# Hongyang-Du/VideoGPA

Hardware: AMD Instinct MI355X
Metric: DPO preference-pair steps/sec, CogVideoX-5B 49f@480x720 (higher is better)
Workload: dtype bf16; 1 GPU; BASELINE configs[1]: CogVideoX-5B T2V full (42 blocks, D=3072, 48x64 heads), 49f x 480x720 -> paired latents [1,2,13,16,60,90], S=17776 tokens, 42 blocks, LoRA r=64 on to_q/to_k/to_v/to_out.0, 1 pair/GPU/step, optimizer step every step; random-init weights; layers=42, pairs_per_gpu=1, parallelism=dp1

## Files before the change

### include/videogpa_hip.h

```cpp
#ifndef VIDEOGPA_HIP_H
#define VIDEOGPA_HIP_H

#include <stddef.h>
#include <stdint.h>

#ifdef __cplusplus
extern "C" {
#endif

typedef struct ihipStream_t* vgpa_stream_t;

#define VGPA_OK 0
#define VGPA_ERR_INVALID (-1)
#define VGPA_ERR_LAUNCH (-2)
#define VGPA_ERR_WORKSPACE (-3)

size_t vgpa_dpo_loss_workspace_bytes(int64_t B);
int32_t vgpa_dpo_loss_fwd(const void* v_win, const void* v_lose, const void* v_win_ref, const void* v_lose_ref,
                          const void* tgt_win, const void* tgt_lose, int64_t B, int64_t N, int64_t stride_pred,
                          int64_t stride_ref, int64_t stride_tgt, int32_t dtype, float beta, float label_smoothing,
                          int32_t loss_type, int32_t flags, float* out5, float* dlogit, float* errs, void* workspace,
                          size_t ws_bytes, vgpa_stream_t stream);
int32_t vgpa_dpo_loss_bwd(const void* v_win, const void* v_lose, const void* tgt_win, const void* tgt_lose, int64_t B,
                          int64_t N, int64_t stride_pred, int64_t stride_tgt, int64_t stride_grad, int32_t dtype, float beta,
                          int32_t flags, const float* dlogit, const float* grad_out, void* grad_win, void* grad_lose,
                          vgpa_stream_t stream);

int32_t vgpa_noise_velocity_paired(const void* x_pair, const void* noise, const int64_t* t, const float* sqrt_abar,
                                   const float* sqrt_1m_abar, int64_t B, int64_t N, int32_t num_train_timesteps,
                                   int32_t dtype, void* x_noisy_pair, void* v_target_pair, vgpa_stream_t stream);

int32_t vgpa_flow_noise_velocity_paired(const void* x_pair, const void* noise, const float* sigma, int64_t B, int64_t N,
                                        int32_t dtype, int32_t xt_f32, void* x_noisy_pair, void* v_target_pair,
                                        vgpa_stream_t stream);

int32_t vgpa_ln_modulate_fwd(const void* x, const float* ln_w, const float* ln_b, const float* shift_v,
                             const float* scale1p_v, const float* shift_t, const float* scale1p_t, int64_t mod_stride,
                             int64_t B, int64_t S, int64_t D, int64_t text_len, float eps, void* out, float* mean,
                             float* rstd, vgpa_stream_t stream);
int32_t vgpa_ln_modulate_bwd(const void* dy, const void* x, const float* mean, const float* rstd, const float* ln_w,
                             const float* scale1p_v, const float* scale1p_t, int64_t mod_stride, int64_t B, int64_t S,
                             int64_t D, int64_t text_len, const void* dres, void* dx, vgpa_stream_t stream);
int32_t vgpa_residual_ln_fwd(const void* x, const void* y, const float* gate_v, const float* gate_t, int64_t gate_stride,
                             const float* ln_w, const float* ln_b, const float* shift_v, const float* scale1p_v,
                             const float* shift_t, const float* scale1p_t, int64_t mod_stride, int64_t B, int64_t S, int64_t D,
                             int64_t text_len, float eps, void* x_new, void* n_out,
                             int64_t n_stride ,
                             float* mean, float* rstd, vgpa_stream_t stream);
int32_t vgpa_residual_ln_bwd(const void* dn, const void* x_new, const float* mean, const float* rstd, const float* ln_w,
                             const float* scale1p_v, const float* scale1p_t, int64_t mod_stride, const float* gate_v,
                             const float* gate_t, int64_t gate_stride, const void* dres, int64_t B, int64_t S, int64_t D,
                             int64_t text_len, void* dx, void* dy, int64_t dy_stride ,
                             vgpa_stream_t stream);
int32_t vgpa_residual_ln_fwd_q8(const void* x, const void* y, const float* gate_v, const float* gate_t, int64_t gate_stride,
                                const float* ln_w, const float* ln_b, const float* shift_v, const float* scale1p_v,
                                const float* shift_t, const float* scale1p_t, int64_t mod_stride, int64_t B, int64_t S, int64_t D,
                                int64_t text_len, float eps, void* x_new, void* q8, float* q8_scale, float* mean, float* rstd,
                                vgpa_stream_t stream);
int32_t vgpa_residual_ln_bwd_q8(const void* dn, const void* x_new, const float* mean, const float* rstd, const float* ln_w,
                                const float* scale1p_v, const float* scale1p_t, int64_t mod_stride, const float* gate_v,
                                const float* gate_t, int64_t gate_stride, const void* dres, int64_t B, int64_t S, int64_t D,
                                int64_t text_len, void* dx, void* dy_q8, float* dy_scale, vgpa_stream_t stream);
int32_t vgpa_gate_residual(const void* x, const void* y, const float* gate_v, const float* gate_t, int64_t mod_stride,
                           int64_t B, int64_t S, int64_t D, int64_t text_len, void* out, vgpa_stream_t stream);
int32_t vgpa_gelu_tanh_fwd(const void* u, int64_t n, void* out, vgpa_stream_t stream);
int32_t vgpa_gelu_tanh_bwd(const void* u, const void* dy, int64_t n, void* du, vgpa_stream_t stream);

int32_t vgpa_qknorm_rope_fwd(const void* q_in, const void* k_in, void* q_out, void* k_out, const int64_t* qin_strides,
                             const int64_t* kin_strides, const int64_t* qout_strides, const int64_t* kout_strides,
                             const float* wq, const float* bq, const float* wk, const float* bk, const float* rope_cos,
                             const float* rope_sin, int64_t text_len, int64_t B, int64_t H, int64_t S, int64_t head_dim,
                             float eps, float q_out_scale, int32_t rope_mode, vgpa_stream_t stream);
int32_t vgpa_qknorm_rope_bwd(const void* dq_out, const void* dk_out, const void* q_in, const void* k_in, void* dq_in,
                             void* dk_in, const int64_t* dqout_strides, const int64_t* dkout_strides,
                             const int64_t* qin_strides, const int64_t* kin_strides, const int64_t* dqin_strides,
                             const int64_t* dkin_strides, const float* wq, const float* wk, const float* rope_cos,
                             const float* rope_sin, int64_t text_len, int64_t B, int64_t H, int64_t S, int64_t head_dim,
                             float eps, int32_t rope_mode, vgpa_stream_t stream);

int32_t vgpa_attn_bwd_delta_res(const void* o, const void* o_res, int32_t res_kind, const void* d_o, const int64_t* o_strides, const int64_t* ores_strides,
                                const int64_t* do_strides, float* delta, int64_t B, int64_t H, int64_t S, int64_t head_dim,
                                vgpa_stream_t stream);
size_t vgpa_attn_bwd_split_workspace_bytes(int64_t B, int64_t H, int64_t S);
int32_t vgpa_attn_bwd_dq_w1(const void* q, const void* k, const void* v, const void* d_o, const float* lse2, const float* delta,
                            void* dq, const int64_t* q_strides, const int64_t* k_strides, const int64_t* v_strides,
                            const int64_t* do_strides, const int64_t* dq_strides, int64_t B, int64_t H, int64_t S, int64_t head_dim,
                            float scale, int32_t split_mode, void* workspace, size_t ws_bytes, vgpa_stream_t stream);
size_t vgpa_attn_fwd_w1_workspace_bytes(int64_t B, int64_t H, int64_t S);
#define VGPA_RES_NONE 0
#define VGPA_RES_BF16 1
#define VGPA_RES_8 2
int32_t vgpa_attn_fwd_w1_res(const void* q, const void* k, const void* v, void* o, void* o_res, int32_t res_kind, float* lse2, const int64_t* q_strides,
                             const int64_t* k_strides, const int64_t* v_strides, const int64_t* o_strides, const int64_t* ores_strides,
                             int64_t B, int64_t H, int64_t S, int64_t head_dim, float scale, int32_t split_mode, void* workspace,
                             size_t ws_bytes, vgpa_stream_t stream);
int32_t vgpa_attn_fwd_online_res(const void* q, const void* k, const void* v, void* o, void* o_res, int32_t res_kind, float* lse2, const int64_t* q_strides,
                                 const int64_t* k_strides, const int64_t* v_strides, const int64_t* o_strides, const int64_t* ores_strides,
                                 int64_t B, int64_t H, int64_t S, int64_t head_dim, float scale, int32_t split_mode, void* workspace,
                                 size_t ws_bytes, vgpa_stream_t stream);
int32_t vgpa_attn_bwd_prep_w1_res(const void* o, const void* o_res, int32_t res_kind, const void* d_o, const float* lse2, const int64_t* o_strides,
                                  const int64_t* ores_strides, const int64_t* do_strides, float* delta, float* stats, int64_t B, int64_t H,
                                  int64_t S, int64_t head_dim, vgpa_stream_t stream);
int32_t vgpa_attn_bwd_dkv_w1(const void* q, const void* k, const void* v, const void* d_o, const float* stats, void* dk, void* dv,
                             const int64_t* q_strides, const int64_t* k_strides, const int64_t* v_strides, const int64_t* do_strides,
                             const int64_t* dk_strides, const int64_t* dv_strides, int64_t B, int64_t H, int64_t S, int64_t head_dim,
                             float scale, int32_t split_mode, void* workspace, size_t ws_bytes, vgpa_stream_t stream);

int32_t vgpa_lora_down(const void* X, int64_t ldx, const void* A, void* T, int64_t ldt, int64_t M, int64_t K, int64_t R,
                       vgpa_stream_t stream);
int32_t vgpa_lora_up_add(void* Y, int64_t ldy, const void* T, int64_t ldt, const void* Bw, int64_t ldb, float s, int64_t M,
                         int64_t N, int64_t rp, int32_t accumulate, vgpa_stream_t stream);
size_t vgpa_lora_grad_workspace_bytes(int64_t M, int64_t P, int64_t Q);
int32_t vgpa_lora_grad_ws(const void* U, int64_t ldu, const void* V, int64_t ldv, float* G, int64_t ldg, float s, int64_t M,
                          int64_t P, int64_t Q, void* workspace, size_t ws_bytes, vgpa_stream_t stream);
int32_t vgpa_lora_ext_refresh(const float* A, const float* B, float s, int64_t r, int64_t K, int64_t Dn, void* a_cat, void* wt_tail, int64_t ld_wt,
                              void* w_tail, int64_t ld_w, void* sbt, vgpa_stream_t stream);

#ifdef VGPA_VARIANTS
int32_t vgpa_gemm_bf16(const void* X, int64_t ldx, const void* W, int64_t ldw, const void* bias, void* C, int64_t ldc, void* aux,
                       int64_t ldaux, int32_t M, int32_t N, int32_t K, int32_t epilogue, vgpa_stream_t stream);
#endif

size_t vgpa_attn128_fwd_workspace_bytes(int64_t B, int64_t H, int64_t Sq);
int32_t vgpa_attn128_fwd(const void* q, const void* k, const void* v, void* o, float* lse2, const int64_t* q_strides, const int64_t* k_strides,
                         const int64_t* v_strides, const int64_t* o_strides, void* o_res8, const int64_t* ores_strides, int64_t B, int64_t H,
                         int64_t Sq, int64_t Skv, float scale, void* workspace, size_t ws_bytes, vgpa_stream_t stream);
size_t vgpa_attn128_fwd_f8_workspace_bytes(int64_t B, int64_t H, int64_t Sq, int64_t Skv);
int32_t vgpa_attn128_fwd_f8(const void* q, const void* k, const void* v, void* o, float* lse2, const int64_t* q_strides, const int64_t* k_strides,
                            const int64_t* v_strides, const int64_t* o_strides, void* o_res8, const int64_t* ores_strides, void* q_deq, void* k_deq,
                            void* v_deq, const int64_t* qd_strides, const int64_t* kd_strides, const int64_t* vd_strides, int64_t B, int64_t H,
                            int64_t Sq, int64_t Skv, float scale, void* workspace, size_t ws_bytes, vgpa_stream_t stream);
size_t vgpa_attn128_bwd_workspace_bytes(int64_t B, int64_t H, int64_t Sq);
int32_t vgpa_attn128_bwd(const void* q, const void* k, const void* v, const void* o, const void* d_o, const float* lse2, void* dq, void* dk,
                         void* dv, const int64_t* q_strides, const int64_t* k_strides, const int64_t* v_strides,
                         const int64_t* o_strides, const int64_t* do_strides, const int64_t* dq_strides, const int64_t* dk_strides,
                         const int64_t* dv_strides, const void* o_res8, const int64_t* ores_strides, int64_t B, int64_t H, int64_t Sq, int64_t Skv,
                         float scale, int32_t dkv_mode, void* workspace, size_t ws_bytes, vgpa_stream_t stream);
int32_t vgpa_attn128_bwd_prescaled(const void* q, const void* k, const void* v, const void* o, const void* d_o, const float* lse2, void* dq, void* dk,
                                   void* dv, const int64_t* q_strides, const int64_t* k_strides, const int64_t* v_strides,
                                   const int64_t* o_strides, const int64_t* do_strides, const int64_t* dq_strides, const int64_t* dk_strides,
                                   const int64_t* dv_strides, const void* o_res8, const int64_t* ores_strides, int64_t B, int64_t H, int64_t Sq, int64_t Skv,
                                   float scale, int32_t dkv_mode, void* workspace, size_t ws_bytes, vgpa_stream_t stream);

int32_t vgpa_wan_ln_mod_fwd(const void* x, int32_t x_dtype, const void* y, const float* gate, float* x_out, const int32_t* gid, const float* ln_w,
                            const float* ln_b, const float* shift, const float* scale, int64_t mod_stride, int64_t rows, int64_t D, float eps,
                            int32_t round_xhat, void* out, int32_t out_dtype, int64_t out_ld, void* q8, float* q8_scale, float* mean, float* rstd,
                            vgpa_stream_t stream);
int32_t vgpa_wan_ln_mod_bwd(const void* dy, int32_t dy_dtype, const void* x, int32_t x_dtype, const float* mean, const float* rstd, const int32_t* gid,
                            const float* ln_w, const float* scale, int64_t mod_stride, int64_t rows, int64_t D, const float* dres, float* dx,
                            const float* gate_prev, void* dy_prev, int64_t ld_dy_prev, vgpa_stream_t stream);
int32_t vgpa_wan_gate_residual(const float* x, const void* y, const int32_t* gid, const float* gate, int64_t mod_stride, int64_t rows, int64_t D, float* out,
                               vgpa_stream_t stream);
int32_t vgpa_wan_gate_bwd(const float* dout, const int32_t* gid, const float* gate, int64_t mod_stride, int64_t rows, int64_t D, void* dy, int64_t ld_dy,
                          vgpa_stream_t stream);
int32_t vgpa_wan_gate_bwd_q8(const float* dout, const int32_t* gid, const float* gate, int64_t mod_stride, int64_t rows, int64_t D, void* q8,
                             float* q8_scale, vgpa_stream_t stream);
int32_t vgpa_wan_rms_rope_fwd(const void* u, int64_t ld_u, const void* w, const float* rope_cos, const float* rope_sin, int64_t L, int64_t head_dim,
                              int64_t rows, int64_t D, float eps, void* out, int64_t ld_out, float* rstd, vgpa_stream_t stream);
int32_t vgpa_wan_rms_rope_bwd(const void* dout, int64_t ld_dout, const void* u, int64_t ld_u, const float* rstd, const void* w, const float* rope_cos,
                              const float* rope_sin, int64_t L, int64_t head_dim, int64_t rows, int64_t D, void* du, int64_t ld_du, vgpa_stream_t stream);

int32_t vgpa_quant_fp8_rows(const void* x, int64_t ldx, void* q, float* scale, int64_t M, int64_t K, vgpa_stream_t stream);
int32_t vgpa_gelu_tanh_fwd_q8(const void* u, int64_t rows, int64_t K, void* q8, float* q8_scale, vgpa_stream_t stream);
int32_t vgpa_gelu_tanh_bwd_q8(const void* u, const void* dy, int64_t rows, int64_t K, void* q8, float* q8_scale, vgpa_stream_t stream);

int32_t vgpa_preprocess_shape(int32_t H, int32_t W, int32_t mode, int32_t* out_h, int32_t* out_w);
size_t vgpa_preprocess_workspace_bytes(int32_t T, int32_t H, int32_t W, int32_t mode);
int32_t vgpa_preprocess_frames(const void* frames, int32_t T, int32_t H, int32_t W, int32_t mode, float* out, void* workspace,
                               size_t ws_bytes, vgpa_stream_t stream);

size_t vgpa_grad_norm_workspace_bytes(void);
int32_t vgpa_grad_norm(const float* grad, int64_t n, float grad_scale, float* norm_out, void* workspace, size_t ws_bytes,
                       vgpa_stream_t stream);
int32_t vgpa_adamw_step(float* param, const float* grad, float* exp_avg, float* exp_avg_sq, int64_t n, float lr, float beta1,
                        float beta2, float eps, float weight_decay, int64_t step, float grad_scale, float max_norm,
                        const float* total_norm, vgpa_stream_t stream);

size_t vgpa_project_points_workspace_bytes(int64_t T, int64_t H, int64_t W);
int32_t vgpa_project_points(const float* pc, const float* colors, const float* conf, float conf_thr,
                            const float* conf_thr_dev , const float* K,
                            const float* E, int32_t e_rows, int64_t N, int64_t T, int64_t H, int64_t W, uint8_t* canvas,
                            float* out_f, void* workspace, size_t ws_bytes, vgpa_stream_t stream);
int32_t vgpa_motion_score(const float* E, int32_t e_rows, int64_t T, float* out, vgpa_stream_t stream);
int32_t vgpa_epipolar_sampson(const float* p1, const float* p2, const int64_t* offsets, int64_t n_pairs, float* err_out,
                              float* F_out, vgpa_stream_t stream);

size_t vgpa_conf_threshold_workspace_bytes(void);
int32_t vgpa_conf_threshold(const float* conf, int64_t N, float conf_thres, float* thr_out, void* workspace, size_t ws_bytes,
                            vgpa_stream_t stream);
size_t vgpa_frame_metric_workspace_bytes(void);
int32_t vgpa_frame_metric(const void* gt, int32_t gt_dtype, int32_t gt_layout, int32_t gt_is_tensor, const void* rep,
                          int32_t rep_dtype, int32_t rep_layout, int32_t rep_is_tensor, int64_t T, int64_t C, int64_t H,
                          int64_t W, int64_t H2, int64_t W2, int32_t psnr, float* out, void* workspace, size_t ws_bytes,
                          vgpa_stream_t stream);
size_t vgpa_frame_ssim_workspace_bytes(int64_t T, int64_t C, int64_t H, int64_t W);
int32_t vgpa_frame_ssim(const void* gt, int32_t gt_dtype, int32_t gt_layout, int32_t gt_is_tensor, const void* rep, int32_t rep_dtype,
                        int32_t rep_layout, int32_t rep_is_tensor, int64_t T, int64_t C, int64_t H, int64_t W, int32_t downsample,
                        float* out_per_frame, float* out_mean, void* workspace, size_t ws_bytes, vgpa_stream_t stream);
int32_t vgpa_frames_to_pm1(const void* src, int32_t dtype, int32_t layout, int32_t is_tensor, int64_t T, int64_t C, int64_t H,
                           int64_t W, int64_t Ho, int64_t Wo, float* out, void* workspace, size_t ws_bytes, vgpa_stream_t stream);
size_t vgpa_mvcs_workspace_bytes(int64_t T);
int32_t vgpa_mvcs(const float* depth, const float* K, int32_t k_dim, const float* E, int32_t e_rows, int64_t T, int64_t H,
                  int64_t W, float* out, void* workspace, size_t ws_bytes, vgpa_stream_t stream);
int32_t vgpa_unproject_depth(const float* depth, const float* K, const float* E, int32_t e_rows, int64_t T, int64_t H,
                             int64_t W, float* world, vgpa_stream_t stream);
int32_t vgpa_pose_decode(const float* pose_enc, int64_t n, float image_h, float image_w, float* ext, float* intr,
                         vgpa_stream_t stream);

int32_t vgpa_conv3x3_f32(const float* x, const float* w_packed, const float* bias, const float* res, const float* res2, float* out,
                         int64_t N, int64_t H, int64_t W, int64_t Cin, int64_t Cout, int64_t stride, int32_t flags,
                         vgpa_stream_t stream);
int32_t vgpa_conv1x1_f32(const float* x, const float* w_packed, const float* bias, float* out, int64_t M, int64_t Cin, int64_t Cout,
                         vgpa_stream_t stream);
int32_t vgpa_dpt_tail_f32(const float* x, const float* xtab, const float* ytab, const float* w1_packed, const float* b1,
                          const float* w2, const float* b2, float* preds, float* conf, int64_t N, int64_t h, int64_t w, int64_t C,
                          int64_t H, int64_t W, int32_t output_dim, int32_t activation, vgpa_stream_t stream);
int32_t vgpa_upsample_bilinear_ac_f32(const float* x, const float* xtab, const float* ytab, float* out, int64_t N, int64_t h,
                                      int64_t w, int64_t C, int64_t H, int64_t W, vgpa_stream_t stream);
int32_t vgpa_attn_small_f32(const float* q, const float* k, const float* v, int64_t stride_b, int64_t stride_h, int64_t stride_s,
                            float* o, int64_t B, int64_t H, int64_t S, int64_t D, float scale, vgpa_stream_t stream);

int32_t vgpa_dino_embed(const void* images, int32_t in_dtype, const float* w_packed, int64_t k_packed, const float* bias,
                        const float* cls_token, const float* register_tokens, const float* pos, void* out, int32_t out_dtype, int64_t N,
                        int64_t H, int64_t W, int64_t patch, int64_t C, int64_t R, vgpa_stream_t stream);
int32_t vgpa_stream_ln_f32(const float* x, const void* y, const float* gamma, const float* ln_w, const float* ln_b, float* x_new, void* n,
                           int32_t n_dtype, int64_t M, int64_t D, float eps, vgpa_stream_t stream);

int32_t vgpa_lpips_input_f32(const float* x, float* out, int64_t N, int64_t H, int64_t W, float shift0, float shift1, float shift2,
                             float scale0, float scale1, float scale2, int32_t flags, vgpa_stream_t stream);
int32_t vgpa_maxpool2x2_f32(const float* x, float* out, int64_t N, int64_t H, int64_t W, int64_t C, int32_t flags, vgpa_stream_t stream);
size_t vgpa_lpips_layer_workspace_bytes(int64_t N, int64_t H, int64_t W, int64_t C);
int32_t vgpa_lpips_layer_f32(const float* f0, const float* f1, const float* w, float* out, double* total, int64_t N, int64_t H, int64_t W,
                             int64_t C, int32_t flags, void* workspace, size_t ws_bytes, vgpa_stream_t stream);

int32_t vgpa_da3_ref_view(const float* x, int64_t B, int64_t S, int64_t N, int64_t C, int32_t strategy, double* metrics, int32_t* ref_idx,
                          vgpa_stream_t stream);
int32_t vgpa_da3_view_gather(const float* a_in, float* a_out, const float* b_in, float* b_out, const int32_t* ref_idx, int32_t inverse, int64_t B,
                             int64_t S, int64_t N, int64_t C, vgpa_stream_t stream);
int32_t vgpa_da3_cam_token(float* x, const float* cam, int32_t per_view, int64_t B, int64_t S, int64_t N, int64_t C, vgpa_stream_t stream);
int32_t vgpa_da3_tap(const float* local_x, const float* x, const float* ln_w, const float* ln_b, float eps, const int32_t* ref_idx, float* feats,
                     float* cam, int64_t B, int64_t S, int64_t N, int64_t C, vgpa_stream_t stream);
int32_t vgpa_da3_pose_decode(const float* pose_enc, int64_t n, float image_h, float image_w, float* ext, float* intr, vgpa_stream_t stream);
int32_t vgpa_dualdpt_aux_tail_f32(const float* x, const float* xtab, const float* ytab, const float* w1_packed, const float* b1,
                                  const float* ln_w, const float* ln_b, float eps, const float* w2, const float* b2, float* preds, float* conf,
                                  int64_t N, int64_t h, int64_t w, int64_t C, int32_t output_dim, vgpa_stream_t stream);

int32_t vgpa_conv3x3_pad_f32(const float* x, const float* w_packed, const float* bias, const float* res, float* out, int64_t N, int64_t H, int64_t W,
                             int64_t Cin, int64_t Cout, int64_t stride, int32_t pad_lo, int32_t pad_hi, vgpa_stream_t stream);
int32_t vgpa_conv3x3x3_causal_f32(const float* x, const float* prev, const float* w_packed, const float* bias, const float* res, float* out, int64_t N,
                                  int64_t T, int64_t H, int64_t W, int64_t Cin, int64_t Cout, vgpa_stream_t stream);
int32_t vgpa_vae_downsample_f32(const float* x, const float* w_packed, const float* bias, float* out, int64_t N, int64_t T, int64_t H, int64_t W,
                                int64_t C, int64_t Cout, int32_t compress_time, vgpa_stream_t stream);
int32_t vgpa_vae_input_f32(const void* x, int32_t in_dtype, float* out, int64_t N, int64_t H, int64_t W, vgpa_stream_t stream);
size_t vgpa_groupnorm_stats_workspace_bytes(int64_t N, int64_t HW, int64_t C, int64_t G);
int32_t vgpa_groupnorm_stats_f32(const float* x, float* stats, int64_t N, int64_t HW, int64_t C, int64_t G, float eps, void* workspace,
                                 size_t ws_bytes, vgpa_stream_t stream);
int32_t vgpa_groupnorm_silu_f32(const float* x, const float* stats, const float* gamma, const float* beta, float* out, int64_t N, int64_t HW,
                                int64_t C, int64_t G, vgpa_stream_t stream);
int32_t vgpa_vae_sample(const float* moments, const void* noise, float scale, void* sample, void* mean, void* logvar, void* std_out,
                        int32_t out_dtype, int64_t N, int64_t hw, int64_t L, vgpa_stream_t stream);

#ifdef __cplusplus
}
#endif
#endif
```

### videogpa_amd/_lib.py

```python
import ctypes
import os

import torch

from ctypes import c_float, c_int32, c_int64, c_size_t, c_void_p

_HERE = os.path.dirname(os.path.abspath(__file__))
LIB_PATH = os.environ.get("VGPA_LIB") or os.path.join(_HERE, "csrc", "libvgpa_hip.so")

P, I64, I32, F32, SZ = c_void_p, c_int64, c_int32, c_float, c_size_t

SIGNATURES = {
    "vgpa_dpo_loss_workspace_bytes": (SZ, [I64]),
    "vgpa_dpo_loss_fwd": (I32, [P, P, P, P, P, P, I64, I64, I64, I64, I64, I32, F32, F32, I32, I32, P, P, P, P, SZ, P]),
    "vgpa_dpo_loss_bwd": (I32, [P, P, P, P, I64, I64, I64, I64, I64, I32, F32, I32, P, P, P, P, P]),
    "vgpa_noise_velocity_paired": (I32, [P, P, P, P, P, I64, I64, I32, I32, P, P, P]),
    "vgpa_flow_noise_velocity_paired": (I32, [P, P, P, I64, I64, I32, I32, P, P, P]),
    "vgpa_ln_modulate_fwd": (I32, [P, P, P, P, P, P, P, I64, I64, I64, I64, I64, F32, P, P, P, P]),
    "vgpa_ln_modulate_bwd": (I32, [P, P, P, P, P, P, P, I64, I64, I64, I64, I64, P, P, P]),
    "vgpa_residual_ln_fwd": (I32, [P, P, P, P, I64, P, P, P, P, P, P, I64, I64, I64, I64, I64, F32, P, P, I64, P, P, P]),
    "vgpa_residual_ln_bwd": (I32, [P, P, P, P, P, P, P, I64, P, P, I64, P, I64, I64, I64, I64, P, P, I64, P]),
    "vgpa_residual_ln_fwd_q8": (I32, [P, P, P, P, I64, P, P, P, P, P, P, I64, I64, I64, I64, I64, F32, P, P, P, P, P, P]),
    "vgpa_residual_ln_bwd_q8": (I32, [P, P, P, P, P, P, P, I64, P, P, I64, P, I64, I64, I64, I64, P, P, P, P]),
    "vgpa_gate_residual": (I32, [P, P, P, P, I64, I64, I64, I64, I64, P, P]),
    "vgpa_gelu_tanh_fwd": (I32, [P, I64, P, P]),
    "vgpa_gelu_tanh_bwd": (I32, [P, P, I64, P, P]),
    "vgpa_qknorm_rope_fwd": (I32, [P, P, P, P, P, P, P, P, P, P, P, P, P, P, I64, I64, I64, I64, I64, F32, F32, I32, P]),
    "vgpa_qknorm_rope_bwd": (I32, [P, P, P, P, P, P, P, P, P, P, P, P, P, P, P, P, I64, I64, I64, I64, I64, F32, I32, P]),
    "vgpa_grad_norm_workspace_bytes": (SZ, []),
    "vgpa_grad_norm": (I32, [P, I64, F32, P, P, SZ, P]),
    "vgpa_adamw_step": (I32, [P, P, P, P, I64, F32, F32, F32, F32, F32, I64, F32, F32, P, P]),
    "vgpa_attn_bwd_delta_res": (I32, [P, P, I32, P, P, P, P, P, I64, I64, I64, I64, P]),
    "vgpa_attn_bwd_dq_w1": (I32, [P, P, P, P, P, P, P, P, P, P, P, P, I64, I64, I64, I64, F32, I32, P, SZ, P]),
    "vgpa_attn_fwd_w1_workspace_bytes": (SZ, [I64, I64, I64]),
    "vgpa_attn_bwd_prep_w1_res": (I32, [P, P, I32, P, P, P, P, P, P, P, I64, I64, I64, I64, P]),
    "vgpa_attn_fwd_w1_res": (I32, [P, P, P, P, P, I32, P, P, P, P, P, P, I64, I64, I64, I64, F32, I32, P, SZ, P]),
    "vgpa_attn_fwd_online_res": (I32, [P, P, P, P, P, I32, P, P, P, P, P, P, I64, I64, I64, I64, F32, I32, P, SZ, P]),
    "vgpa_attn_bwd_dkv_w1": (I32, [P, P, P, P, P, P, P, P, P, P, P, P, P, I64, I64, I64, I64, F32, I32, P, SZ, P]),
    "vgpa_attn_bwd_split_workspace_bytes": (SZ, [I64, I64, I64]),
    "vgpa_lora_down": (I32, [P, I64, P, P, I64, I64, I64, I64, P]),
    "vgpa_lora_up_add": (I32, [P, I64, P, I64, P, I64, F32, I64, I64, I64, I32, P]),
    "vgpa_lora_grad_workspace_bytes": (SZ, [I64, I64, I64]),
    "vgpa_lora_grad_ws": (I32, [P, I64, P, I64, P, I64, F32, I64, I64, I64, P, SZ, P]),
    "vgpa_lora_ext_refresh": (I32, [P, P, F32, I64, I64, I64, P, P, I64, P, I64, P, P]),
    "vgpa_attn128_fwd_workspace_bytes": (SZ, [I64, I64, I64]),
    "vgpa_attn128_fwd": (I32, [P, P, P, P, P, P, P, P, P, P, P, I64, I64, I64, I64, F32, P, SZ, P]),
    "vgpa_attn128_fwd_f8_workspace_bytes": (SZ, [I64, I64, I64, I64]),
    "vgpa_attn128_fwd_f8": (I32, [P] * 17 + [I64, I64, I64, I64, F32, P, SZ, P]),
    "vgpa_attn128_bwd_workspace_bytes": (SZ, [I64, I64, I64]),
    "vgpa_attn128_bwd": (I32, [P] * 19 + [I64, I64, I64, I64, F32, I32, P, SZ, P]),
    "vgpa_attn128_bwd_prescaled": (I32, [P] * 19 + [I64, I64, I64, I64, F32, I32, P, SZ, P]),
    "vgpa_wan_ln_mod_fwd": (I32, [P, I32, P, P, P, P, P, P, P, P, I64, I64, I64, F32, I32, P, I32, I64, P, P, P, P, P]),
    "vgpa_wan_ln_mod_bwd": (I32, [P, I32, P, I32, P, P, P, P, P, I64, I64, I64, P, P, P, P, I64, P]),
    "vgpa_wan_gate_residual": (I32, [P, P, P, P, I64, I64, I64, P, P]),
    "vgpa_wan_gate_bwd": (I32, [P, P, P, I64, I64, I64, P, I64, P]),
    "vgpa_wan_gate_bwd_q8": (I32, [P, P, P, I64, I64, I64, P, P, P]),
    "vgpa_wan_rms_rope_fwd": (I32, [P, I64, P, P, P, I64, I64, I64, I64, F32, P, I64, P, P]),
    "vgpa_wan_rms_rope_bwd": (I32, [P, I64, P, I64, P, P, P, P, I64, I64, I64, I64, P, I64, P]),
    "vgpa_quant_fp8_rows": (I32, [P, I64, P, P, I64, I64, P]),
    "vgpa_gelu_tanh_fwd_q8": (I32, [P, I64, I64, P, P, P]),
    "vgpa_gelu_tanh_bwd_q8": (I32, [P, P, I64, I64, P, P, P]),
    "vgpa_preprocess_shape": (I32, [I32, I32, I32, P, P]),
    "vgpa_preprocess_workspace_bytes": (SZ, [I32, I32, I32, I32]),
    "vgpa_preprocess_frames": (I32, [P, I32, I32, I32, I32, P, P, SZ, P]),
    "vgpa_project_points_workspace_bytes": (SZ, [I64, I64, I64]),
    "vgpa_project_points": (I32, [P, P, P, F32, P, P, P, I32, I64, I64, I64, I64, P, P, P, SZ, P]),
    "vgpa_conf_threshold_workspace_bytes": (SZ, []),
    "vgpa_conf_threshold": (I32, [P, I64, F32, P, P, SZ, P]),
    "vgpa_frame_metric_workspace_bytes": (SZ, []),
    "vgpa_frame_metric": (I32, [P, I32, I32, I32, P, I32, I32, I32, I64, I64, I64, I64, I64, I64, I32, P, P, SZ, P]),
    "vgpa_frame_ssim_workspace_bytes": (SZ, [I64, I64, I64, I64]),
    "vgpa_frame_ssim": (I32, [P, I32, I32, I32, P, I32, I32, I32, I64, I64, I64, I64, I32, P, P, P, SZ, P]),
    "vgpa_frames_to_pm1": (I32, [P, I32, I32, I32, I64, I64, I64, I64, I64, I64, P, P, SZ, P]),
    "vgpa_mvcs_workspace_bytes": (SZ, [I64]),
    "vgpa_mvcs": (I32, [P, P, I32, P, I32, I64, I64, I64, P, P, SZ, P]),
    "vgpa_unproject_depth": (I32, [P, P, P, I32, I64, I64, I64, P, P]),
    "vgpa_pose_decode": (I32, [P, I64, F32, F32, P, P, P]),
    "vgpa_motion_score": (I32, [P, I32, I64, P, P]),
    "vgpa_epipolar_sampson": (I32, [P, P, P, I64, P, P, P]),
    "vgpa_conv3x3_f32": (I32, [P, P, P, P, P, P, I64, I64, I64, I64, I64, I64, I32, P]),
    "vgpa_conv1x1_f32": (I32, [P, P, P, P, I64, I64, I64, P]),
    "vgpa_dpt_tail_f32": (I32, [P, P, P, P, P, P, P, P, P, I64, I64, I64, I64, I64, I64, I32, I32, P]),
    "vgpa_upsample_bilinear_ac_f32": (I32, [P, P, P, P, I64, I64, I64, I64, I64, I64, P]),
    "vgpa_attn_small_f32": (I32, [P, P, P, I64, I64, I64, P, I64, I64, I64, I64, F32, P]),
    "vgpa_dino_embed": (I32, [P, I32, P, I64, P, P, P, P, P, I32, I64, I64, I64, I64, I64, I64, P]),
    "vgpa_stream_ln_f32": (I32, [P, P, P, P, P, P, P, I32, I64, I64, F32, P]),
    "vgpa_lpips_input_f32": (I32, [P, P, I64, I64, I64, F32, F32, F32, F32, F32, F32, I32, P]),
    "vgpa_maxpool2x2_f32": (I32, [P, P, I64, I64, I64, I64, I32, P]),
    "vgpa_lpips_layer_workspace_bytes": (SZ, [I64, I64, I64, I64]),
    "vgpa_lpips_layer_f32": (I32, [P, P, P, P, P, I64, I64, I64, I64, I32, P, SZ, P]),
    "vgpa_da3_ref_view": (I32, [P, I64, I64, I64, I64, I32, P, P, P]),
    "vgpa_da3_view_gather": (I32, [P, P, P, P, P, I32, I64, I64, I64, I64, P]),
    "vgpa_da3_cam_token": (I32, [P, P, I32, I64, I64, I64, I64, P]),
    "vgpa_da3_tap": (I32, [P, P, P, P, F32, P, P, P, I64, I64, I64, I64, P]),
    "vgpa_da3_pose_decode": (I32, [P, I64, F32, F32, P, P, P]),
    "vgpa_dualdpt_aux_tail_f32": (I32, [P, P, P, P, P, P, P, F32, P, P, P, P, I64, I64, I64, I64, I32, P]),
    "vgpa_conv3x3_pad_f32": (I32, [P, P, P, P, P, I64, I64, I64, I64, I64, I64, I32, I32, P]),
    "vgpa_conv3x3x3_causal_f32": (I32, [P, P, P, P, P, P, I64, I64, I64, I64, I64, I64, P]),
    "vgpa_vae_downsample_f32": (I32, [P, P, P, P, I64, I64, I64, I64, I64, I64, I32, P]),
    "vgpa_vae_input_f32": (I32, [P, I32, P, I64, I64, I64, P]),
    "vgpa_groupnorm_stats_workspace_bytes": (SZ, [I64, I64, I64, I64]),
    "vgpa_groupnorm_stats_f32": (I32, [P, P, I64, I64, I64, I64, F32, P, SZ, P]),
    "vgpa_groupnorm_silu_f32": (I32, [P, P, P, P, P, I64, I64, I64, I64, P]),
    "vgpa_vae_sample": (I32, [P, P, F32, P, P, P, P, I32, I64, I64, I64, P]),
}

OPTIONAL_SIGNATURES = {
    "vgpa_gemm_bf16": (I32, [P, I64, P, I64, P, P, I64, P, I64, I32, I32, I32, I32, P]),
}

_ERR = {-1: "invalid argument", -2: "kernel launch failed", -3: "workspace too small"}
_lib = None


def load():
    global _lib
    if _lib is None:
        if not os.path.exists(LIB_PATH):
            raise RuntimeError(
                f"videogpa_amd: HIP library not built ({LIB_PATH} missing). Run `python -m videogpa_amd.build` "
                "(or __graft_entry__.build()). There is no CPU / PyTorch fallback.")
        lib = ctypes.CDLL(LIB_PATH)
        for name, (res, args) in SIGNATURES.items():
            fn = getattr(lib, name)
            fn.restype = res
            fn.argtypes = args
        for name, (res, args) in OPTIONAL_SIGNATURES.items():
            fn = getattr(lib, name, None)
            if fn is not None:
                fn.restype = res
                fn.argtypes = args
        _lib = lib
    return _lib


def _conv(a):
    if a is None:
        return None
    if hasattr(a, "data_ptr"):
        return a.data_ptr()
    return a


def call(name, *args):
    fn = getattr(load(), name)
    rc = fn(*[_conv(a) for a in args])
    if rc != 0:
        raise RuntimeError(f"{name} failed: {_ERR.get(rc, rc)}")


def query(name, *args):
    return getattr(load(), name)(*args)


def has(name):
    return hasattr(load(), name)
```

### videogpa_amd/csrc/attention_w1.hip

```cpp
#include <type_traits>

#include "attn_w1.h"

#define W1_DQ_PART_FLOATS (256 * HD)
#define W1_DKV_PART_FLOATS (2 * 256 * HD)

template <bool SPLIT>
__global__ __launch_bounds__(256, 1) void attn_bwd_dq_w1_kernel(const bf16_t* __restrict__ Q, const bf16_t* __restrict__ K,
                                                                  const bf16_t* __restrict__ V, const bf16_t* __restrict__ dO,
                                                                  const float* __restrict__ LSE2, const float* __restrict__ DELTA,
                                                                  bf16_t* __restrict__ dQ, TStride sq, TStride sk, TStride sv, TStride sdo,
                                                                  TStride sdq, int S, int H, int n_qt, float scale, int task0, int nsplit,
                                                                  float* __restrict__ part) {
    constexpr int QB = 2;
    __shared__ __attribute__((aligned(1024))) uint8_t lds[W1_RING_BYTES];
    int vid, chunk;
    w1_task<SPLIT>(task0, nsplit, vid, chunk);
    const int bh = vid / n_qt, qt = vid % n_qt;
    const int b = bh / H, h = bh % H;
    const int lane = threadIdx.x & 63, hi = lane >> 5;
    const int wave = __builtin_amdgcn_readfirstlane((int)threadIdx.x >> 6);
    const int q0 = (qt * 4 + wave) * (32 * QB);

    bf16x8_t qf[QB][4], dof[QB][4];
    f32x16_t cs[QB], cd[QB];
#pragma unroll
    for (int j = 0; j < QB; ++j) {
        load_row_frags(Q + ((size_t)b * sq.b + (size_t)h * sq.h), sq.s, q0 + 32 * j, S, lane, qf[j]);
        load_row_frags(dO + ((size_t)b * sdo.b + (size_t)h * sdo.h), sdo.s, q0 + 32 * j, S, lane, dof[j]);
        int qc = q0 + 32 * j + (lane & 31);
        qc = qc < S ? qc : S - 1;
        const float nl = -LSE2[(int64_t)bh * S + qc], nd = -DELTA[(int64_t)bh * S + qc];
#pragma unroll
        for (int i = 0; i < 16; ++i) { cs[j][i] = nl; cd[j][i] = nd; }
    }
#pragma unroll
    for (int j = 0; j < QB; ++j) { frags_arrived(qf[j]); frags_arrived(dof[j]); }

    const W1Range tr = w1_split_range(S, chunk, nsplit, SPLIT);
    const int tb = tr.tb, nt = tr.nt;

    w1_zero_slot(lds, 3 * W1_SLOT_BYTES, 2);
    __syncthreads();

    const bf16_t* Kb = K + ((size_t)b * sk.b + (size_t)h * sk.h);
    const bf16_t* Vb = V + ((size_t)b * sv.b + (size_t)h * sv.h);
    const W1Rsrc krs = w1_rsrc(Kb, ((uint32_t)(S - 1) * sk.s + (uint32_t)HD) * 2u);
    const W1Rsrc vrs = w1_rsrc(Vb, ((uint32_t)(S - 1) * sv.s + (uint32_t)HD) * 2u);
    uint32_t kvo[2], vvo[2];
    w1_dma_offsets<HD>(wave, lane, sk.s, kvo);
    w1_dma_offsets<HD>(wave, lane, sv.s, vvo);
    const uint32_t kstep = __builtin_amdgcn_readfirstlane(64u * sk.s * 2u), vstep = __builtin_amdgcn_readfirstlane(64u * sv.s * 2u);
    const uint32_t wbase = __builtin_amdgcn_readfirstlane((uint32_t)(uintptr_t)(__attribute__((address_space(3))) uint8_t*)lds + (uint32_t)wave * 2048u);
    u32x4_t voff = {kvo[0] + (uint32_t)tb * kstep, kvo[1] + (uint32_t)tb * kstep, vvo[0] + (uint32_t)tb * vstep, vvo[1] + (uint32_t)tb * vstep};
    w1_prime<HD>(wbase, krs, vrs, voff, kstep, vstep);

    const u32x8_t la8 = w1_read_offsets<HD>(lane);
    const u32x16_t qf0 = w1_pack4(qf[0][0], qf[0][1], qf[0][2], qf[0][3]), qf1 = w1_pack4(qf[1][0], qf[1][1], qf[1][2], qf[1][3]);
    const u32x16_t do0 = w1_pack4(dof[0][0], dof[0][1], dof[0][2], dof[0][3]), do1 = w1_pack4(dof[1][0], dof[1][1], dof[1][2], dof[1][3]);
    const uint32_t niter = (uint32_t)(nt - tb + 1);
    f32x16_t dq[QB][2];
    uint32_t t0, t1, t2;
    asm volatile(
#include "w1_dq_loop.inc"
        : "=&s"(t0), "=&s"(t1), "=&s"(t2), "={a[0:15]}"(dq[0][0]), "={a[16:31]}"(dq[0][1]), "={a[32:47]}"(dq[1][0]), "={a[48:63]}"(dq[1][1]),
          "+{v[232:235]}"(voff)
        : [rk] "s"(krs.w), [rv] "s"(vrs.w), [kstep] "s"(kstep), [vstep] "s"(vstep), [wbase] "s"(wbase), [niter] "s"(niter), "{a[64:79]}"(qf0),
          "{a[80:95]}"(qf1), "{a[96:111]}"(do0), "{a[112:127]}"(do1), "{v[160:175]}"(cs[0]), "{v[176:191]}"(cs[1]), "{v[192:207]}"(cd[0]), "{v[208:223]}"(cd[1]), "{v[224:231]}"(la8)
        : "memory", "scc",
#include "w1_dq_clobbers.inc"
    );
#pragma unroll
    for (int j = 0; j < QB; ++j) { asm volatile("" : "+v"(dq[j][0])); asm volatile("" : "+v"(dq[j][1])); }

    if (SPLIT) {
        float* pb = part + ((size_t)(vid - task0) * nsplit + chunk) * W1_DQ_PART_FLOATS;
#pragma unroll
        for (int j = 0; j < QB; ++j) {
            const int r = wave * (32 * QB) + 32 * j + (lane & 31);
#pragma unroll
            for (int db = 0; db < 2; ++db)
#pragma unroll
                for (int g = 0; g < 4; ++g) {
                    const f32x4_t w = {dq[j][db][4 * g], dq[j][db][4 * g + 1], dq[j][db][4 * g + 2], dq[j][db][4 * g + 3]};
                    *reinterpret_cast<f32x4_t*>(pb + r * HD + db * 32 + 8 * g + 4 * hi) = w;
                }
        }
        return;
    }
#pragma unroll
    for (int j = 0; j < QB; ++j) {
        const int q = q0 + 32 * j + (lane & 31);
        if (q < S) {
            bf16_t* op = dQ + ((size_t)b * sdq.b + (size_t)h * sdq.h + (size_t)q * sdq.s);
#pragma unroll
            for (int db = 0; db < 2; ++db)
#pragma unroll
                for (int gp = 0; gp < 2; ++gp) {
                    u32x2_t w[2];
#pragma unroll
                    for (int e = 0; e < 2; ++e) {
                        const int g = 2 * gp + e;
                        w[e][0] = pack_bf16x2(dq[j][db][4 * g] * scale, dq[j][db][4 * g + 1] * scale);
                        w[e][1] = pack_bf16x2(dq[j][db][4 * g + 2] * scale, dq[j][db][4 * g + 3] * scale);
                    }
                    *reinterpret_cast<u32x4_t*>(op + db * 32 + 8 * (2 * gp + hi)) = pair_rows8(w[0], w[1]);
                }
        }
    }
}

#include "w1_fwd_knobs.inc"
#define W1_FWD_PART_FLOATS (256 * (HD + 2))
#define W1_FWD_MIN_S 128

__device__ __forceinline__ u32x2_t w1_residual4(const float* x, u32x2_t packed) {
    u32x2_t r;
    r[0] = pack_bf16x2(x[0] - __uint_as_float(packed[0] << 16), x[1] - __uint_as_float(packed[0] & 0xffff0000u));
    r[1] = pack_bf16x2(x[2] - __uint_as_float(packed[1] << 16), x[3] - __uint_as_float(packed[1] & 0xffff0000u));
    return r;
}

template <bool SPLIT>
__global__ __launch_bounds__(256, 1) void attn_fwd_w1_kernel(const bf16_t* __restrict__ Q, const bf16_t* __restrict__ K, const bf16_t* __restrict__ V,
                                                               bf16_t* __restrict__ O, float* __restrict__ LSE2, const unsigned* __restrict__ KMAX2,
                                                               int* __restrict__ flags, TStride sq, TStride sk, TStride sv, TStride so, int S, int H,
                                                               int n_qt, int task0, int nsplit, float* __restrict__ part, void* __restrict__ ORES,
                                                               TStride sor, int res_kind) {
    constexpr int QB = 2;
    __shared__ __attribute__((aligned(1024))) uint8_t lds[W1_RING_BYTES];
    int vid, chunk;
    w1_task<SPLIT>(task0, nsplit, vid, chunk);
    const int bh = vid / n_qt, qt = vid % n_qt;
    const int b = bh / H, h = bh % H;
    const int lane = threadIdx.x & 63, hi = lane >> 5;
    const int wave = __builtin_amdgcn_readfirstlane((int)threadIdx.x >> 6);
    const int q0 = (qt * 4 + wave) * (32 * QB);

    bf16x8_t qf[QB][4];
    float nm[QB];
    const float kmax = sqrtf(__uint_as_float(KMAX2[bh]));
#pragma unroll
    for (int j = 0; j < QB; ++j) load_row_frags(Q + ((size_t)b * sq.b + (size_t)h * sq.h), sq.s, q0 + 32 * j, S, lane, qf[j]);
#pragma unroll
    for (int j = 0; j < QB; ++j) {
        frags_arrived(qf[j]);
        float a = 0.f;
#pragma unroll
        for (int ks = 0; ks < 4; ++ks) {
            float f[8];
            frag_to_f32(qf[j][ks], f);
#pragma unroll
            for (int i = 0; i < 8; ++i) a += f[i] * f[i];
        }
        a += other_half(a);
        nm[j] = sqrtf(a) * kmax * 1.0009765625f;
    }
    {
        const bf16_t* Ks = K + ((size_t)b * sk.b + (size_t)h * sk.h);
        const uint32_t step = (uint32_t)S / W1_SAMPLE_KEYS;
        float ms[QB];
#pragma unroll
        for (int j = 0; j < QB; ++j) ms[j] = -INFINITY;
#pragma unroll
        for (int kb = 0; kb < W1_SAMPLE_KEYS / 32; ++kb) {
            bf16x8_t kf[4];
            load_row_frags(Ks, sk.s * step, 32 * kb, W1_SAMPLE_KEYS, lane, kf);
            frags_arrived(kf);
#pragma unroll
            for (int j = 0; j < QB; ++j) {
                f32x16_t acc = {0.f, 0.f, 0.f, 0.f, 0.f, 0.f, 0.f, 0.f, 0.f, 0.f, 0.f, 0.f, 0.f, 0.f, 0.f, 0.f};
#pragma unroll
                for (int ks = 0; ks < 4; ++ks) acc = mfma32(kf[ks], qf[j][ks], acc);
                float m = acc[0];
#pragma unroll
                for (int i = 1; i < 16; ++i) m = fmaxf(m, acc[i]);
                ms[j] = fmaxf(ms[j], fmaxf(m, other_half(m)));
            }
        }
#pragma unroll
        for (int j = 0; j < QB; ++j) nm[j] = -fminf(nm[j], ms[j] + W1_SAMPLE_UP);
    }

    const W1Range tr = w1_split_range(S, chunk, nsplit, SPLIT);
    const int tb = tr.tb, nt = tr.nt;

    w1_zero_slot(lds, 3 * W1_SLOT_BYTES + W1_TILE_BYTES, 2);
    __syncthreads();

    const bf16_t* Kb = K + ((size_t)b * sk.b + (size_t)h * sk.h);
    const bf16_t* Vb = V + ((size_t)b * sv.b + (size_t)h * sv.h);
    const W1Rsrc krs = w1_rsrc(Kb, ((uint32_t)(S - 1) * sk.s + (uint32_t)HD) * 2u);
    const W1Rsrc vrs = w1_rsrc(Vb, ((uint32_t)(S - 1) * sv.s + (uint32_t)HD) * 2u);
    uint32_t kvo[2], vvo[2];
    w1_dma_offsets<HD>(wave, lane, sk.s, kvo);
    w1_dma_offsets<HD>(wave, lane, sv.s, vvo);
    const uint32_t kstep = __builtin_amdgcn_readfirstlane(64u * sk.s * 2u), vstep = __builtin_amdgcn_readfirstlane(64u * sv.s * 2u);
    const uint32_t wbase = __builtin_amdgcn_readfirstlane((uint32_t)(uintptr_t)(__attribute__((address_space(3))) uint8_t*)lds + (uint32_t)wave * 2048u);
    u32x4_t voff = {kvo[0] + (uint32_t)tb * kstep, kvo[1] + (uint32_t)tb * kstep, vvo[0] + (uint32_t)tb * vstep, vvo[1] + (uint32_t)tb * vstep};
    w1_prime<HD>(wbase, krs, vrs, voff, kstep, vstep);

    const u32x8_t la8 = w1_read_offsets<HD>(lane);
    const u32x16_t qf0 = w1_pack4(qf[0][0], qf[0][1], qf[0][2], qf[0][3]), qf1 = w1_pack4(qf[1][0], qf[1][1], qf[1][2], qf[1][3]);
    const uint32_t niter = (uint32_t)(nt - tb + 1);
    const int kend = nt * TILE < S ? nt * TILE : S;
    const uint32_t krem = (uint32_t)(kend - tb * TILE);
    const uint32_t hi4 = 4u * (uint32_t)hi;
#if W1_FWD_MFSUM
    const uint32_t sel = (lane == 0 || lane == 32 || lane == 17 || lane == 49) ? 0x3f803f80u : 0u;
#define W1_FWD_SEL_IN , "{v158}"(sel)
#else
#define W1_FWD_SEL_IN
#endif
    f32x16_t o[QB][2];
    u32x8_t lv;
    uint32_t t0, t1, t2, t3;
    uint64_t c0, c1;
    asm volatile(
#include "w1_fwd_loop.inc"
        : "=&s"(t0), "=&s"(t1), "=&s"(t2), "=&s"(t3), [c0] "=&s"(c0), [c1] "=&s"(c1), "={a[0:15]}"(o[0][0]), "={a[16:31]}"(o[0][1]), "={a[32:47]}"(o[1][0]), "={a[48:63]}"(o[1][1]),
          "={v[128:135]}"(lv), "+{v[152:155]}"(voff)
        : [rk] "s"(krs.w), [rv] "s"(vrs.w), [kstep] "s"(kstep), [vstep] "s"(vstep), [wbase] "s"(wbase), [niter] "s"(niter), [krem] "s"(krem),
          "{a[64:79]}"(qf0), "{a[80:95]}"(qf1), "{v136}"(nm[0]), "{v137}"(nm[1]), "{v[144:151]}"(la8), "{v156}"(hi4) W1_FWD_SEL_IN
        : "memory", "scc", "vcc",
#include "w1_fwd_clobbers.inc"
    );
#pragma unroll
    for (int j = 0; j < QB; ++j) { asm volatile("" : "+v"(o[j][0])); asm volatile("" : "+v"(o[j][1])); }

    float l[QB];
#pragma unroll
    for (int j = 0; j < QB; ++j) {
#if W1_FWD_MFSUM
        const float s0 = __shfl(__uint_as_float(lv[4 * j]), lane & 15, 64), s1 = __shfl(__uint_as_float(lv[4 * j + 1]), lane & 15, 64);
        l[j] = (lane & 16) ? s1 : s0;
#else
        const float a = (__uint_as_float(lv[4 * j]) + __uint_as_float(lv[4 * j + 1])) + (__uint_as_float(lv[4 * j + 2]) + __uint_as_float(lv[4 * j + 3]));
        l[j] = a + other_half(a);
#endif
    }
    if (SPLIT) {
        float* pb = part + ((size_t)(vid - task0) * nsplit + chunk) * W1_FWD_PART_FLOATS;
#pragma unroll
        for (int j = 0; j < QB; ++j) {
            const int r = wave * (32 * QB) + 32 * j + (lane & 31);
#pragma unroll
            for (int db = 0; db < 2; ++db)
#pragma unroll
                for (int g = 0; g < 4; ++g) {
                    const f32x4_t w = {o[j][db][4 * g], o[j][db][4 * g + 1], o[j][db][4 * g + 2], o[j][db][4 * g + 3]};
                    *reinterpret_cast<f32x4_t*>(pb + r * HD + db * 32 + 8 * g + 4 * hi) = w;
                }
            if (hi == 0) { pb[256 * HD + r] = -nm[j]; pb[256 * HD + 256 + r] = l[j]; }
        }
        return;
    }
    bool bad = false;
#pragma unroll
    for (int j = 0; j < QB; ++j) {
        const int q = q0 + 32 * j + (lane & 31);
        if (q < S) {
            bad = bad || w1_strip_bad(l[j], -nm[j], o[j]);
            const float inv = 1.f / l[j];
            bf16_t* op = O + ((size_t)b * so.b + (size_t)h * so.h + (size_t)q * so.s);
            const size_t ro = (size_t)b * sor.b + (size_t)h * sor.h + (size_t)q * sor.s;
#pragma unroll
            for (int db = 0; db < 2; ++db)
#pragma unroll
                for (int gp = 0; gp < 2; ++gp) {
                    u32x2_t w[2], rw[2];
                    uint32_t rb[2];
#pragma unroll
                    for (int e = 0; e < 2; ++e) {
                        float x[4];
                        w[e] = w1_pack_bf16x4(o[j][db], 2 * gp + e, inv, x);
                        if (res_kind == VGPA_RES_8) rb[e] = res8_pack4(x, w[e]);
                        else if (res_kind == VGPA_RES_BF16) rw[e] = w1_residual4(x, w[e]);
                    }
                    const int d0 = db * 32 + 8 * (2 * gp + hi);
                    *reinterpret_cast<u32x4_t*>(op + d0) = pair_rows8(w[0], w[1]);
                    if (res_kind == VGPA_RES_8) *reinterpret_cast<u32x2_t*>((uint8_t*)ORES + ro + d0) = pair_rows8_dword(rb[0], rb[1]);
                    else if (res_kind == VGPA_RES_BF16) *reinterpret_cast<u32x4_t*>((bf16_t*)ORES + ro + d0) = pair_rows8(rw[0], rw[1]);
                }
            if (hi == 0) LSE2[(int64_t)bh * S + q] = -nm[j] + __builtin_amdgcn_logf(l[j]);
        }
    }
#ifdef W1_CLOCKS
    if (threadIdx.x == 0) flags[vid] = (int)(c1 - c0);
    (void)bad;
#else
    if (__any(bad) && lane == 0) flags[vid] = 1;
#endif
}

__global__ __launch_bounds__(256) void w1_fwd_merge_kernel(const float* __restrict__ part, int nsplit, int task0, int n_qt, bf16_t* __restrict__ O, TStride so,
                                                             float* __restrict__ LSE2, int* __restrict__ flags, int S, int H, void* __restrict__ ORES,
                                                             TStride sor, int res_kind) {
    const int lane = threadIdx.x & 63, r = (blockIdx.x & 63) * 4 + (threadIdx.x >> 6), tl = blockIdx.x >> 6;
    const int vid = task0 + tl, bh = vid / n_qt, qt = vid % n_qt;
    const int q = qt * 256 + r;
    if (q >= S) return;
    const float* pb = part + (size_t)tl * nsplit * W1_FWD_PART_FLOATS;
    float acc = 0.f, L = 0.f;
    for (int c = 0; c < nsplit; ++c) {
        const float* pc = pb + (size_t)c * W1_FWD_PART_FLOATS;
        acc += pc[r * HD + lane];
        L += pc[256 * HD + 256 + r];
    }
    const int b = bh / H, h = bh % H;
    const float x = acc / L;
    const bf16_t xb = f32_to_bf16(x);
    O[(size_t)b * so.b + (size_t)h * so.h + (size_t)q * so.s + lane] = xb;
    const size_t ro = (size_t)b * sor.b + (size_t)h * sor.h + (size_t)q * sor.s + lane;
    if (res_kind == VGPA_RES_8) ((uint8_t*)ORES)[ro] = (uint8_t)res8_byte(x, xb);
    else if (res_kind == VGPA_RES_BF16) ((bf16_t*)ORES)[ro] = f32_to_bf16(x - bf16_to_f32(xb));
    const bool obad = __any(!(fabsf(acc) < INFINITY));
    if (lane == 0) {
        LSE2[(int64_t)bh * S + q] = pb[256 * HD + r] + __builtin_amdgcn_logf(L);
        if (w1_stats_bad(L, pb[256 * HD + r]) || obad) flags[vid] = 1;
    }
}

template <bool SPLIT>
__global__ __launch_bounds__(256, 1) void attn_bwd_dkv_w1_kernel(const bf16_t* __restrict__ Q, const bf16_t* __restrict__ K,
                                                                   const bf16_t* __restrict__ V, const bf16_t* __restrict__ dO,
                                                                   const float* __restrict__ STATS, bf16_t* __restrict__ dK, bf16_t* __restrict__ dV,
                                                                   TStride sq, TStride sk, TStride sv, TStride sdo, TStride sdk, TStride sdv, int S,
                                                                   int H, int n_kt, float kscale, int task0, int nsplit, float* __restrict__ part) {
    constexpr int KB = 2;
    __shared__ __attribute__((aligned(1024))) uint8_t lds[W1_RING_BYTES + W1_SLOTS * W1_STAT_BYTES];
    int vid, chunk;
    w1_task<SPLIT>(task0, nsplit, vid, chunk);
    const int bh = vid / n_kt, kt = vid % n_kt;
    const int b = bh / H, h = bh % H;
    const int lane = threadIdx.x & 63, hi = lane >> 5;
    const int wave = __builtin_amdgcn_readfirstlane((int)threadIdx.x >> 6);
    const int k0 = (kt * 4 + wave) * (32 * KB);

    bf16x8_t kf[KB][4], vf[KB][4];
#pragma unroll
    for (int j = 0; j < KB; ++j) {
        load_row_frags(K + ((size_t)b * sk.b + (size_t)h * sk.h), sk.s, k0 + 32 * j, S, lane, kf[j]);
        load_row_frags(V + ((size_t)b * sv.b + (size_t)h * sv.h), sv.s, k0 + 32 * j, S, lane, vf[j]);
    }
#pragma unroll
    for (int j = 0; j < KB; ++j) { frags_arrived(kf[j]); frags_arrived(vf[j]); }

    const W1Range tr = w1_split_range(S, chunk, nsplit, SPLIT);
    const int tb = tr.tb, nt = tr.nt;

    {
        const u32x4_t z = {0u, 0u, 0u, 0u};
#pragma unroll
        for (int i = 0; i < 4; ++i) *reinterpret_cast<u32x4_t*>(lds + 3 * W1_SLOT_BYTES + i * 4096 + threadIdx.x * 16) = z;
    }
    __syncthreads();

    const bf16_t* Qb = Q + ((size_t)b * sq.b + (size_t)h * sq.h);
    const bf16_t* dOb = dO + ((size_t)b * sdo.b + (size_t)h * sdo.h);
    const W1Rsrc qrs = w1_rsrc(Qb, ((uint32_t)(S - 1) * sq.s + (uint32_t)HD) * 2u);
    const W1Rsrc dors = w1_rsrc(dOb, ((uint32_t)(S - 1) * sdo.s + (uint32_t)HD) * 2u);
    const W1Rsrc strs = w1_rsrc(STATS + (int64_t)bh * 2 * S, (uint32_t)(2 * S) * 4u);
    uint32_t qvo[2], dvo[2];
    w1_dma_offsets<HD>(wave, lane, sq.s, qvo);
    w1_dma_offsets<HD>(wave, lane, sdo.s, dvo);
    const uint32_t qstep = __builtin_amdgcn_readfirstlane(64u * sq.s * 2u), dstep = __builtin_amdgcn_readfirstlane(64u * sdo.s * 2u);
    const uint32_t lds0 = (uint32_t)(uintptr_t)(__attribute__((address_space(3))) uint8_t*)lds;
    const uint32_t wbase = __builtin_amdgcn_readfirstlane(lds0 + (uint32_t)wave * 2048u);
    const uint32_t sbase = __builtin_amdgcn_readfirstlane(lds0 + (uint32_t)W1_RING_BYTES + (uint32_t)wave * 256u);
    const uint32_t srow = (uint32_t)(16 * wave + (lane & 15)), splane = (uint32_t)((lane >> 4) & 1);
    uint32_t svo = (splane * (uint32_t)S + srow + (uint32_t)tb * 64u) * 4u;
    u32x4_t voff = {qvo[0] + (uint32_t)tb * qstep, qvo[1] + (uint32_t)tb * qstep, dvo[0] + (uint32_t)tb * dstep, dvo[1] + (uint32_t)tb * dstep};
#pragma unroll
    for (int i = 0; i < 2; ++i) {
        const uint32_t dst = wbase + (uint32_t)i * W1_SLOT_BYTES;
        w1_dma(dst, qrs, voff[0], 0u);
        w1_dma(dst + 1024u, qrs, voff[1], 0u);
        w1_dma(dst + W1_TILE_BYTES, dors, voff[2], 0u);
        w1_dma(dst + W1_TILE_BYTES + 1024u, dors, voff[3], 0u);
        w1_dma4(sbase + (uint32_t)i * W1_STAT_BYTES, strs, svo, 0u);
        voff[0] += qstep; voff[1] += qstep; voff[2] += dstep; voff[3] += dstep;
        svo += 256u;
    }

    const u32x8_t la8 = w1_read_offsets<HD>(lane);
    const uint32_t sread = lds0 + (uint32_t)W1_RING_BYTES + 16u * (uint32_t)hi;
    const u32x16_t kf0 = w1_pack4(kf[0][0], kf[0][1], kf[0][2], kf[0][3]), kf1 = w1_pack4(kf[1][0], kf[1][1], kf[1][2], kf[1][3]);
    const u32x16_t vf0 = w1_pack4(vf[0][0], vf[0][1], vf[0][2], vf[0][3]), vf1 = w1_pack4(vf[1][0], vf[1][1], vf[1][2], vf[1][3]);
    const uint32_t niter = (uint32_t)(nt - tb + 1);
    f32x16_t dk[KB][2], dv[KB][2];
    uint32_t t0, t1;
    asm volatile(
#include "w1_dkv_loop.inc"
        : "=&s"(t0), "=&s"(t1), "={a[0:15]}"(dk[0][0]), "={a[16:31]}"(dk[0][1]), "={a[32:47]}"(dk[1][0]), "={a[48:63]}"(dk[1][1]),
          "={a[64:79]}"(dv[0][0]), "={a[80:95]}"(dv[0][1]), "={a[96:111]}"(dv[1][0]), "={a[112:127]}"(dv[1][1]), "+{v[232:235]}"(voff), "+{v236}"(svo)
        : [rq] "s"(qrs.w), [rdo] "s"(dors.w), [rst] "s"(strs.w), [qstep] "s"(qstep), [dstep] "s"(dstep), [wbase] "s"(wbase), [sbase] "s"(sbase),
          [niter] "s"(niter), "{a[128:143]}"(kf0), "{a[144:159]}"(kf1), "{a[160:175]}"(vf0), "{a[176:191]}"(vf1), "{v[224:231]}"(la8), "{v237}"(sread)
        : "memory", "scc",
#include "w1_dkv_clobbers.inc"
    );
#pragma unroll
    for (int j = 0; j < KB; ++j)
#pragma unroll
        for (int db = 0; db < 2; ++db) { asm volatile("" : "+v"(dk[j][db])); asm volatile("" : "+v"(dv[j][db])); }

    if (SPLIT) {
        float* pb = part + ((size_t)(vid - task0) * nsplit + chunk) * W1_DKV_PART_FLOATS;
#pragma unroll
        for (int j = 0; j < KB; ++j) {
            const int r = wave * (32 * KB) + 32 * j + (lane & 31);
            w1_store_part_row(pb, r, dk[j], hi);
            w1_store_part_row(pb + 256 * HD, r, dv[j], hi);
        }
        return;
    }
#pragma unroll
    for (int j = 0; j < KB; ++j) {
        const int k = k0 + 32 * j + (lane & 31);
        if (k < S) {
            w1_store_bf16_row(dK + ((size_t)b * sdk.b + (size_t)h * sdk.h + (size_t)k * sdk.s), dk[j], kscale, hi);
            w1_store_bf16_row(dV + ((size_t)b * sdv.b + (size_t)h * sdv.h + (size_t)k * sdv.s), dv[j], 1.f, hi);
        }
    }
}

__global__ __launch_bounds__(256) void w1_dkv_merge_kernel(const float* __restrict__ part, int nsplit, int task0, int n_kt, bf16_t* __restrict__ dK,
                                                             bf16_t* __restrict__ dV, TStride sdk, TStride sdv, int S, int H, float kscale) {
    const int lane = threadIdx.x & 63;
    const int r = ((int)blockIdx.x % 64) * 4 + (threadIdx.x >> 6), tl = (int)blockIdx.x / 64;
    const int vid = task0 + tl, bh = vid / n_kt, kt = vid % n_kt;
    const int key = kt * 256 + r;
    if (key >= S) return;
    const float* pb = part + (size_t)tl * nsplit * W1_DKV_PART_FLOATS + r * HD + lane;
    float ak = 0.f, av = 0.f;
    for (int c = 0; c < nsplit; ++c) {
        ak += pb[(size_t)c * W1_DKV_PART_FLOATS];
        av += pb[(size_t)c * W1_DKV_PART_FLOATS + 256 * HD];
    }
    const int b = bh / H, h = bh % H;
    dK[(size_t)b * sdk.b + (size_t)h * sdk.h + (size_t)key * sdk.s + lane] = f32_to_bf16(ak * kscale);
    dV[(size_t)b * sdv.b + (size_t)h * sdv.h + (size_t)key * sdv.s + lane] = f32_to_bf16(av);
}

__global__ __launch_bounds__(256) void w1_bwd_prep_kernel(const bf16_t* __restrict__ dO, const bf16_t* __restrict__ O, const float* __restrict__ LSE2,
                                                            TStride sdo, TStride so, int S, int H, int64_t total , float* __restrict__ delta,
                                                            float* __restrict__ stats, const void* __restrict__ ORES, TStride sor, int res_kind) {
    const int64_t gid = (int64_t)blockIdx.x * 256 + threadIdx.x;
    const int64_t row = gid >> 3;
    const int c8 = (int)(gid & 7);
    float acc = 0.f;
    int64_t bh = 0;
    int q = 0;
    if (row < total) {
        q = (int)(row % S);
        bh = row / S;
        const int h = (int)(bh % H), b = (int)(bh / H);
        float a[8], o[8];
        unpack8(*reinterpret_cast<const u32x4_t*>(dO + ((size_t)b * sdo.b + (size_t)h * sdo.h + (size_t)q * sdo.s + c8 * 8)), a);
        const u32x4_t ob = *reinterpret_cast<const u32x4_t*>(O + ((size_t)b * so.b + (size_t)h * so.h + (size_t)q * so.s + c8 * 8));
        const size_t ro = (size_t)b * sor.b + (size_t)h * sor.h + (size_t)q * sor.s + c8 * 8;
        if (res_kind == VGPA_RES_8) {
            unpack8_res8(ob, *reinterpret_cast<const u32x2_t*>((const uint8_t*)ORES + ro), o);
        } else {
            unpack8(ob, o);
            if (res_kind == VGPA_RES_BF16) {
                float r[8];
                unpack8(*reinterpret_cast<const u32x4_t*>((const bf16_t*)ORES + ro), r);
#pragma unroll
                for (int j = 0; j < 8; ++j) o[j] += r[j];
            }
        }
#pragma unroll
        for (int j = 0; j < 8; ++j) acc += a[j] * o[j];
    }
    acc += __shfl_xor(acc, 1, 64);
    acc += __shfl_xor(acc, 2, 64);
    acc += __shfl_xor(acc, 4, 64);
    if (row < total && c8 == 0) {
        delta[row] = acc;
        stats[bh * 2 * S + q] = -LSE2[row];
        stats[bh * 2 * S + S + q] = -acc;
    }
}

__global__ __launch_bounds__(256) void w1_dq_merge_kernel(const float* __restrict__ part, int nsplit, int task0, int n_qt, int rows_per_task,
                                                            bf16_t* __restrict__ dQ, TStride sdq, int S, int H, float scale) {
    const int lane = threadIdx.x & 63, rows4 = rows_per_task >> 2;
    const int r = ((int)blockIdx.x % rows4) * 4 + (threadIdx.x >> 6), tl = (int)blockIdx.x / rows4;
    const int vid = task0 + tl, bh = vid / n_qt, qt = vid % n_qt;
    const int q = qt * rows_per_task + r;
    if (q >= S) return;
    const float* pb = part + (size_t)tl * nsplit * rows_per_task * HD + r * HD + lane;
    float acc = 0.f;
    for (int c = 0; c < nsplit; ++c) acc += pb[(size_t)c * rows_per_task * HD];
    const int b = bh / H, h = bh % H;
    dQ[(size_t)b * sdq.b + (size_t)h * sdq.h + (size_t)q * sdq.s + lane] = f32_to_bf16(acc * scale);
}

#define W1_MAX_SPLIT 16
static inline int64_t w1_slots() { return wg_slots() / 2; }

extern "C" {


size_t vgpa_attn_bwd_split_workspace_bytes(int64_t B, int64_t H, int64_t S) {
    if (B <= 0 || H <= 0 || S <= 0) return 0;
    const int64_t tasks = (S + 255) / 256 * B * H;
    const size_t part = W1_DKV_PART_FLOATS > W1_DQ_PART_FLOATS ? W1_DKV_PART_FLOATS : W1_DQ_PART_FLOATS;
    return (size_t)max_split_parts(tasks, W1_MAX_SPLIT, w1_slots()) * part * sizeof(float);
}

int32_t vgpa_attn_bwd_dq_w1(const void* q, const void* k, const void* v, const void* d_o, const float* lse2, const float* delta, void* dq,
                            const int64_t* q_strides, const int64_t* k_strides, const int64_t* v_strides, const int64_t* do_strides,
                            const int64_t* dq_strides, int64_t B, int64_t H, int64_t S, int64_t head_dim, float scale, int32_t split_mode,
                            void* workspace, size_t ws_bytes, hipStream_t stream) {
    if (!q || !k || !v || !d_o || !lse2 || !delta || !dq || head_dim != HD || B <= 0 || H <= 0 || S <= 0 || S > (1 << 24)) return VGPA_ERR_INVALID;
    if (!view_ok(q_strides, B, H, S, HD) || !view_ok(k_strides, B, H, S, HD) || !view_ok(v_strides, B, H, S, HD) || !view_ok(do_strides, B, H, S, HD) ||
        !view_ok(dq_strides, B, H, S, HD) || !al16(q) || !al16(k) || !al16(v) || !al16(d_o) || !al16(dq) || (workspace && !al16(workspace)))
        return VGPA_ERR_INVALID;
    const int rows = 256;
    W1Plan pl;
    const int32_t rc = plan_w1(B, H, S, split_mode, W1_MAX_SPLIT, w1_slots(), W1_DQ_PART_FLOATS * sizeof(float), workspace, ws_bytes, 0, &pl);
    if (rc) return rc;
    const int n_t = pl.n_t;
    const TailSplit& p = pl.p;
    if (p.n_main > 0) {
        VGPA_LAUNCH((attn_bwd_dq_w1_kernel<false>), dim3((unsigned)p.n_main), dim3(256), 0, stream, (const bf16_t*)q, (const bf16_t*)k,
                    (const bf16_t*)v, (const bf16_t*)d_o, lse2, delta, (bf16_t*)dq, mk(q_strides), mk(k_strides), mk(v_strides), mk(do_strides),
                    mk(dq_strides), (int)S, (int)H, n_t, scale, 0, 1, (float*)nullptr);
        VGPA_CHECK_LAUNCH();
    }
    if (p.n_tail > 0) {
        VGPA_LAUNCH((attn_bwd_dq_w1_kernel<true>), dim3((unsigned)(p.n_tail * p.nsplit)), dim3(256), 0, stream, (const bf16_t*)q, (const bf16_t*)k,
                    (const bf16_t*)v, (const bf16_t*)d_o, lse2, delta, (bf16_t*)dq, mk(q_strides), mk(k_strides), mk(v_strides), mk(do_strides),
                    mk(dq_strides), (int)S, (int)H, n_t, scale, (int)p.n_main, p.nsplit, (float*)workspace);
        VGPA_CHECK_LAUNCH();
        VGPA_LAUNCH(w1_dq_merge_kernel, dim3((unsigned)(p.n_tail * (rows / 4))), dim3(256), 0, stream, (const float*)workspace, p.nsplit, (int)p.n_main, n_t,
                    rows, (bf16_t*)dq, mk(dq_strides), (int)S, (int)H, scale);
        VGPA_CHECK_LAUNCH();
    }
    return VGPA_OK;
}


int32_t vgpa_attn_bwd_prep_w1_res(const void* o, const void* o_res, int32_t res_kind, const void* d_o, const float* lse2, const int64_t* o_strides,
                                  const int64_t* ores_strides, const int64_t* do_strides, float* delta, float* stats, int64_t B, int64_t H, int64_t S,
                                  int64_t head_dim, hipStream_t stream) {
    if (!o || !d_o || !lse2 || !delta || !stats || head_dim != HD || B <= 0 || H <= 0 || S <= 0 || S > (1 << 24)) return VGPA_ERR_INVALID;
    if (!view_ok(o_strides, B, H, S, HD) || !view_ok(do_strides, B, H, S, HD) || !al16(o) || !al16(d_o)) return VGPA_ERR_INVALID;
    if (o_res && (!view_ok(ores_strides, B, H, S, HD) || !al16(o_res) || (res_kind != VGPA_RES_BF16 && res_kind != VGPA_RES_8))) return VGPA_ERR_INVALID;
    const int64_t total = B * H * S;
    VGPA_LAUNCH(w1_bwd_prep_kernel, dim3((unsigned)((total * 8 + 255) / 256)), dim3(256), 0, stream, (const bf16_t*)d_o, (const bf16_t*)o, lse2,
                mk(do_strides), mk(o_strides), (int)S, (int)H, total, delta, stats, o_res, o_res ? mk(ores_strides) : mk(o_strides),
                o_res ? (int)res_kind : VGPA_RES_NONE);
    VGPA_CHECK_LAUNCH();
    return VGPA_OK;
}

int32_t vgpa_attn_bwd_dkv_w1(const void* q, const void* k, const void* v, const void* d_o, const float* stats, void* dk, void* dv,
                             const int64_t* q_strides, const int64_t* k_strides, const int64_t* v_strides, const int64_t* do_strides,
                             const int64_t* dk_strides, const int64_t* dv_strides, int64_t B, int64_t H, int64_t S, int64_t head_dim, float scale,
                             int32_t split_mode, void* workspace, size_t ws_bytes, hipStream_t stream) {
    (void)scale;
    if (!q || !k || !v || !d_o || !stats || !dk || !dv || head_dim != HD || B <= 0 || H <= 0 || S <= 0 || S > (1 << 24)) return VGPA_ERR_INVALID;
    if (!view_ok(q_strides, B, H, S, HD) || !view_ok(k_strides, B, H, S, HD) || !view_ok(v_strides, B, H, S, HD) || !view_ok(do_strides, B, H, S, HD) ||
        !view_ok(dk_strides, B, H, S, HD) || !view_ok(dv_strides, B, H, S, HD) || !al16(q) || !al16(k) || !al16(v) || !al16(d_o) || !al16(dk) ||
        !al16(dv) || (workspace && !al16(workspace)))
        return VGPA_ERR_INVALID;
    const float kscale = 0.6931471805599453f;
    W1Plan pl;
    const int32_t rc = plan_w1(B, H, S, split_mode, W1_MAX_SPLIT, w1_slots(), W1_DKV_PART_FLOATS * sizeof(float), workspace, ws_bytes, 0, &pl);
    if (rc) return rc;
    const int n_t = pl.n_t;
    const TailSplit& p = pl.p;
    if (p.n_main > 0) {
        VGPA_LAUNCH((attn_bwd_dkv_w1_kernel<false>), dim3((unsigned)p.n_main), dim3(256), 0, stream, (const bf16_t*)q, (const bf16_t*)k, (const bf16_t*)v,
                    (const bf16_t*)d_o, stats, (bf16_t*)dk, (bf16_t*)dv, mk(q_strides), mk(k_strides), mk(v_strides), mk(do_strides), mk(dk_strides),
                    mk(dv_strides), (int)S, (int)H, n_t, kscale, 0, 1, (float*)nullptr);
        VGPA_CHECK_LAUNCH();
    }
    if (p.n_tail > 0) {
        VGPA_LAUNCH((attn_bwd_dkv_w1_kernel<true>), dim3((unsigned)(p.n_tail * p.nsplit)), dim3(256), 0, stream, (const bf16_t*)q, (const bf16_t*)k,
                    (const bf16_t*)v, (const bf16_t*)d_o, stats, (bf16_t*)dk, (bf16_t*)dv, mk(q_strides), mk(k_strides), mk(v_strides), mk(do_strides),
                    mk(dk_strides), mk(dv_strides), (int)S, (int)H, n_t, kscale, (int)p.n_main, p.nsplit, (float*)workspace);
        VGPA_CHECK_LAUNCH();
        VGPA_LAUNCH(w1_dkv_merge_kernel, dim3((unsigned)(p.n_tail * 64)), dim3(256), 0, stream, (const float*)workspace, p.nsplit, (int)p.n_main, n_t,
                    (bf16_t*)dk, (bf16_t*)dv, mk(dk_strides), mk(dv_strides), (int)S, (int)H, kscale);
        VGPA_CHECK_LAUNCH();
    }
    return VGPA_OK;
}


static inline size_t fwd_w1_ws_head(int64_t B, int64_t H, int64_t tasks) { return (((size_t)(B * H) + (size_t)tasks) * 4 + 255) / 256 * 256; }
size_t vgpa_attn_fwd_w1_workspace_bytes(int64_t B, int64_t H, int64_t S) {
    const int64_t tasks = (S + 255) / 256 * B * H;
    return fwd_w1_ws_head(B, H, tasks) + (size_t)max_split_parts(tasks, W1_MAX_SPLIT, w1_slots()) * W1_FWD_PART_FLOATS * sizeof(float);
}
static int32_t fwd_w1_impl(const void* q, const void* k, const void* v, void* o, void* o_res, int32_t res_kind, float* lse2, const int64_t* q_strides,
                           const int64_t* k_strides, const int64_t* v_strides, const int64_t* o_strides, const int64_t* ores_strides, int64_t B,
                           int64_t H, int64_t S, int64_t head_dim, float scale, int32_t split_mode, void* workspace, size_t ws_bytes,
                           hipStream_t stream, bool force_online) {
    (void)scale;
    if (!q || !k || !v || !o || !lse2 || !workspace || head_dim != HD || B <= 0 || H <= 0 || S <= 0 || S > (1 << 24)) return VGPA_ERR_INVALID;
    if (!view_ok(q_strides, B, H, S, HD) || !view_ok(k_strides, B, H, S, HD) || !view_ok(v_strides, B, H, S, HD) || !view_ok(o_strides, B, H, S, HD) ||
        !al16(q) || !al16(k) || !al16(v) || !al16(o) || !al16(workspace))
        return VGPA_ERR_INVALID;
    if (o_res && (!view_ok(ores_strides, B, H, S, HD) || !al16(o_res) || (res_kind != VGPA_RES_BF16 && res_kind != VGPA_RES_8))) return VGPA_ERR_INVALID;
    void* ores = o_res;
    const int rk = o_res ? (int)res_kind : VGPA_RES_NONE;
    const TStride sor = o_res ? mk(ores_strides) : mk(o_strides);
    if (B * H > 65535) return VGPA_ERR_INVALID;
    const size_t head = fwd_w1_ws_head(B, H, (S + 255) / 256 * B * H);
    W1Plan pl;
    const int32_t rc = plan_w1(B, H, S, force_online ? 0 : split_mode, W1_MAX_SPLIT, w1_slots(), W1_FWD_PART_FLOATS * sizeof(float), workspace, ws_bytes, head, &pl);
    if (rc) return rc;
    if (ws_bytes < head) return VGPA_ERR_WORKSPACE;
    const int n_qt = pl.n_t;
    const int64_t tasks = pl.tasks;
    const TailSplit& p = pl.p;
    unsigned* kmax2 = (unsigned*)workspace;
    int* flags = (int*)workspace + B * H;
    float* part = (float*)((char*)workspace + head);
    if (S < W1_FWD_MIN_S || force_online) {
        if (hipMemsetAsync(workspace, 0xff, head, stream) != hipSuccess) return VGPA_ERR_LAUNCH;
        return vgpa_internal_attn_fwd_redo(q, k, v, o, lse2, mk(q_strides), mk(k_strides), mk(v_strides), mk(o_strides), (int)S, (int)H, n_qt, tasks,
                                           flags, stream, ores, sor, rk);
    }
    if (hipMemsetAsync(workspace, 0, head, stream) != hipSuccess) return VGPA_ERR_LAUNCH;
    VGPA_LAUNCH((w1_kmax_kernel<HD / 8>), dim3(16, (unsigned)(B * H)), dim3(256), 0, stream, (const bf16_t*)k, mk(k_strides), (int)S, (int)H, kmax2);
    VGPA_CHECK_LAUNCH();
    if (p.n_main > 0) {
        VGPA_LAUNCH((attn_fwd_w1_kernel<false>), dim3((unsigned)p.n_main), dim3(256), 0, stream, (const bf16_t*)q, (const bf16_t*)k, (const bf16_t*)v,
                    (bf16_t*)o, lse2, (const unsigned*)kmax2, flags, mk(q_strides), mk(k_strides), mk(v_strides), mk(o_strides), (int)S, (int)H, n_qt, 0, 1,
                    (float*)nullptr, ores, sor, rk);
        VGPA_CHECK_LAUNCH();
    }
    if (p.n_tail > 0) {
        VGPA_LAUNCH((attn_fwd_w1_kernel<true>), dim3((unsigned)(p.n_tail * p.nsplit)), dim3(256), 0, stream, (const bf16_t*)q, (const bf16_t*)k,
                    (const bf16_t*)v, (bf16_t*)o, lse2, (const unsigned*)kmax2, flags, mk(q_strides), mk(k_strides), mk(v_strides), mk(o_strides), (int)S,
                    (int)H, n_qt, (int)p.n_main, p.nsplit, part, ores, sor, rk);
        VGPA_CHECK_LAUNCH();
        VGPA_LAUNCH(w1_fwd_merge_kernel, dim3((unsigned)(p.n_tail * 64)), dim3(256), 0, stream, (const float*)part, p.nsplit, (int)p.n_main, n_qt, (bf16_t*)o,
                    mk(o_strides), lse2, flags, (int)S, (int)H, ores, sor, rk);
        VGPA_CHECK_LAUNCH();
    }
    return vgpa_internal_attn_fwd_redo(q, k, v, o, lse2, mk(q_strides), mk(k_strides), mk(v_strides), mk(o_strides), (int)S, (int)H, n_qt, tasks, flags, stream,
                                       ores, sor, rk);
}
int32_t vgpa_attn_fwd_w1_res(const void* q, const void* k, const void* v, void* o, void* o_res, int32_t res_kind, float* lse2, const int64_t* q_strides,
                             const int64_t* k_strides, const int64_t* v_strides, const int64_t* o_strides, const int64_t* ores_strides, int64_t B,
                             int64_t H, int64_t S, int64_t head_dim, float scale, int32_t split_mode, void* workspace, size_t ws_bytes,
                             hipStream_t stream) {
    return fwd_w1_impl(q, k, v, o, o_res, res_kind, lse2, q_strides, k_strides, v_strides, o_strides, ores_strides, B, H, S, head_dim, scale, split_mode, workspace,
                       ws_bytes, stream, false);
}
int32_t vgpa_attn_fwd_online_res(const void* q, const void* k, const void* v, void* o, void* o_res, int32_t res_kind, float* lse2, const int64_t* q_strides,
                                 const int64_t* k_strides, const int64_t* v_strides, const int64_t* o_strides, const int64_t* ores_strides, int64_t B,
                                 int64_t H, int64_t S, int64_t head_dim, float scale, int32_t split_mode, void* workspace, size_t ws_bytes,
                                 hipStream_t stream) {
    return fwd_w1_impl(q, k, v, o, o_res, res_kind, lse2, q_strides, k_strides, v_strides, o_strides, ores_strides, B, H, S, head_dim, scale, split_mode, workspace,
                       ws_bytes, stream, true);
}

}
```

### videogpa_amd/csrc/qknorm.hip

```cpp
#include "common.h"

struct QStride { int64_t b, h, s; };

__device__ __forceinline__ float group8_sum(float v) {
    v += __shfl_xor(v, 1, 64);
    v += __shfl_xor(v, 2, 64);
    v += __shfl_xor(v, 4, 64);
    return v;
}

__global__ __launch_bounds__(256) void qknorm_rope_fwd_kernel(const bf16_t* __restrict__ q_in, const bf16_t* __restrict__ k_in,
                                                                bf16_t* __restrict__ q_out, bf16_t* __restrict__ k_out, QStride si_q,
                                                                QStride si_k, QStride so_q, QStride so_k, const float* __restrict__ wq,
                                                                const float* __restrict__ bq, const float* __restrict__ wk,
                                                                const float* __restrict__ bk, const float* __restrict__ rope_cos,
                                                                const float* __restrict__ rope_sin, int text_len, int B, int H, int S,
                                                                float eps, float q_out_scale, int rope_mode) {
    const int64_t nvec = (int64_t)B * S * H;
    const int64_t gid = (int64_t)blockIdx.x * 256 + threadIdx.x;
    const int64_t vid = gid >> 3;
    const int c8 = (int)(gid & 7);
    if (vid >= 2 * nvec) return;
    const int which = vid >= nvec;
    uint32_t r = (uint32_t)(which ? vid - nvec : vid);
    const int h = (int)(r % (uint32_t)H); r /= (uint32_t)H;
    const int s = (int)(r % (uint32_t)S);
    const int b = (int)(r / (uint32_t)S);
    const bf16_t* ip = which ? (k_in + b * si_k.b + h * si_k.h + (int64_t)s * si_k.s) : (q_in + b * si_q.b + h * si_q.h + (int64_t)s * si_q.s);
    bf16_t* op = which ? (k_out + b * so_k.b + h * so_k.h + (int64_t)s * so_k.s) : (q_out + b * so_q.b + h * so_q.h + (int64_t)s * so_q.s);
    const float* w = which ? wk : wq;
    const float* bb = which ? bk : bq;
    float x[8];
    unpack8(*reinterpret_cast<const u32x4_t*>(ip + c8 * 8), x);
    float sum = 0.f;
#pragma unroll
    for (int j = 0; j < 8; ++j) sum += x[j];
    const float mean = group8_sum(sum) * (1.f / 64.f);
    float sq = 0.f;
#pragma unroll
    for (int j = 0; j < 8; ++j) { const float d = x[j] - mean; sq += d * d; }
    const float rstd = rsqrtf(group8_sum(sq) * (1.f / 64.f) + eps);
    float y[8];
#pragma unroll
    for (int j = 0; j < 8; ++j) y[j] = (x[j] - mean) * rstd * w[c8 * 8 + j] + bb[c8 * 8 + j];
    if (rope_cos && rope_mode == 1) {
        const bool on = s >= text_len;
        const float* cp = rope_cos + (int64_t)(on ? s - text_len : 0) * 64 + c8 * 8;
        const float* sp = rope_sin + (int64_t)(on ? s - text_len : 0) * 64 + c8 * 8;
        const float sgn = (c8 & 2) ? 1.f : -1.f;
#pragma unroll
        for (int j = 0; j < 8; ++j) {
            const float partner = __shfl_xor(y[j], 2, 64);
            if (on) y[j] = y[j] * cp[j] + sgn * partner * sp[j];
        }
    } else if (rope_cos && s >= text_len) {
        const float* cp = rope_cos + (int64_t)(s - text_len) * 64 + c8 * 8;
        const float* sp = rope_sin + (int64_t)(s - text_len) * 64 + c8 * 8;
#pragma unroll
        for (int j = 0; j < 8; j += 2) {
            const float a = y[j], bq2 = y[j + 1];
            y[j] = a * cp[j] - bq2 * sp[j];
            y[j + 1] = bq2 * cp[j + 1] + a * sp[j + 1];
        }
    }
    if (!which) {
#pragma unroll
        for (int j = 0; j < 8; ++j) y[j] *= q_out_scale;
    }
    *reinterpret_cast<u32x4_t*>(op + c8 * 8) = pack8(y);
}

__global__ __launch_bounds__(256) void qknorm_rope_bwd_kernel(const bf16_t* __restrict__ dq_out, const bf16_t* __restrict__ dk_out,
                                                                const bf16_t* __restrict__ q_in, const bf16_t* __restrict__ k_in,
                                                                bf16_t* __restrict__ dq_in, bf16_t* __restrict__ dk_in, QStride sg_q,
                                                                QStride sg_k, QStride si_q, QStride si_k, QStride sd_q, QStride sd_k,
                                                                const float* __restrict__ wq, const float* __restrict__ wk,
                                                                const float* __restrict__ rope_cos, const float* __restrict__ rope_sin,
                                                                int text_len, int B, int H, int S, float eps, int rope_mode) {
    const int64_t nvec = (int64_t)B * S * H;
    const int64_t gid = (int64_t)blockIdx.x * 256 + threadIdx.x;
    const int64_t vid = gid >> 3;
    const int c8 = (int)(gid & 7);
    if (vid >= 2 * nvec) return;
    const int which = vid >= nvec;
    uint32_t r = (uint32_t)(which ? vid - nvec : vid);
    const int h = (int)(r % (uint32_t)H); r /= (uint32_t)H;
    const int s = (int)(r % (uint32_t)S);
    const int b = (int)(r / (uint32_t)S);
    const QStride sg = which ? sg_k : sg_q, si = which ? si_k : si_q, sd = which ? sd_k : sd_q;
    const bf16_t* gp = (which ? dk_out : dq_out) + b * sg.b + h * sg.h + (int64_t)s * sg.s;
    const bf16_t* ip = (which ? k_in : q_in) + b * si.b + h * si.h + (int64_t)s * si.s;
    bf16_t* op = (which ? dk_in : dq_in) + b * sd.b + h * sd.h + (int64_t)s * sd.s;
    const float* w = which ? wk : wq;
    float g[8], x[8];
    unpack8(*reinterpret_cast<const u32x4_t*>(gp + c8 * 8), g);
    unpack8(*reinterpret_cast<const u32x4_t*>(ip + c8 * 8), x);
    if (rope_cos && rope_mode == 1) {
        const bool on = s >= text_len;
        const int64_t row = (int64_t)(on ? s - text_len : 0) * 64;
        const float* cp = rope_cos + row + c8 * 8;
        const float* spp = rope_sin + row + (c8 ^ 2) * 8;
        const float sgn = (c8 & 2) ? -1.f : 1.f;
#pragma unroll
        for (int j = 0; j < 8; ++j) {
            const float partner = __shfl_xor(g[j], 2, 64);
            if (on) g[j] = g[j] * cp[j] + sgn * partner * spp[j];
        }
    } else if (rope_cos && s >= text_len) {
        const float* cp = rope_cos + (int64_t)(s - text_len) * 64 + c8 * 8;
        const float* sp = rope_sin + (int64_t)(s - text_len) * 64 + c8 * 8;
#pragma unroll
        for (int j = 0; j < 8; j += 2) {
            const float d0 = g[j], d1 = g[j + 1];
            g[j] = d0 * cp[j] + d1 * sp[j + 1];
            g[j + 1] = d1 * cp[j + 1] - d0 * sp[j];
        }
    }
    float sum = 0.f;
#pragma unroll
    for (int j = 0; j < 8; ++j) sum += x[j];
    const float mean = group8_sum(sum) * (1.f / 64.f);
    float sq = 0.f;
#pragma unroll
    for (int j = 0; j < 8; ++j) { x[j] -= mean; sq += x[j] * x[j]; }
    const float rstd = rsqrtf(group8_sum(sq) * (1.f / 64.f) + eps);
    float s1 = 0.f, s2 = 0.f;
#pragma unroll
    for (int j = 0; j < 8; ++j) {
        x[j] *= rstd;
        g[j] *= w[c8 * 8 + j];
        s1 += g[j];
        s2 += g[j] * x[j];
    }
    const float c1 = group8_sum(s1) * (1.f / 64.f), c2 = group8_sum(s2) * (1.f / 64.f);
#pragma unroll
    for (int j = 0; j < 8; ++j) g[j] = rstd * (g[j] - c1 - x[j] * c2);
    *reinterpret_cast<u32x4_t*>(op + c8 * 8) = pack8(g);
}

static inline bool qs_ok(const int64_t* st) { return st && (st[0] % 8 == 0) && (st[1] % 8 == 0) && (st[2] % 8 == 0); }
static inline QStride qmk(const int64_t* st) { QStride t; t.b = st[0]; t.h = st[1]; t.s = st[2]; return t; }

extern "C" {

int32_t vgpa_qknorm_rope_fwd(const void* q_in, const void* k_in, void* q_out, void* k_out, const int64_t* qin_strides,
                             const int64_t* kin_strides, const int64_t* qout_strides, const int64_t* kout_strides, const float* wq,
                             const float* bq, const float* wk, const float* bk, const float* rope_cos, const float* rope_sin,
                             int64_t text_len, int64_t B, int64_t H, int64_t S, int64_t head_dim, float eps, float q_out_scale,
                             int32_t rope_mode, hipStream_t stream) {
    if (!q_in || !k_in || !q_out || !k_out || !wq || !bq || !wk || !bk || head_dim != 64 || B <= 0 || H <= 0 || S <= 0) return VGPA_ERR_INVALID;
    if (!qs_ok(qin_strides) || !qs_ok(kin_strides) || !qs_ok(qout_strides) || !qs_ok(kout_strides)) return VGPA_ERR_INVALID;
    if ((rope_cos == nullptr) != (rope_sin == nullptr) || text_len < 0 || text_len > S || (rope_mode != 0 && rope_mode != 1)) return VGPA_ERR_INVALID;
    const int64_t threads = 2 * B * S * H * 8;
    if (2 * B * S * H >= ((int64_t)1 << 31) || threads / 256 >= ((int64_t)1 << 31)) return VGPA_ERR_INVALID;
    VGPA_LAUNCH(qknorm_rope_fwd_kernel, dim3((unsigned)((threads + 255) / 256)), dim3(256), 0, stream, (const bf16_t*)q_in,
                       (const bf16_t*)k_in, (bf16_t*)q_out, (bf16_t*)k_out, qmk(qin_strides), qmk(kin_strides), qmk(qout_strides),
                       qmk(kout_strides), wq, bq, wk, bk, rope_cos, rope_sin, (int)text_len, (int)B, (int)H, (int)S, eps, q_out_scale, (int)rope_mode);
    VGPA_CHECK_LAUNCH();
    return VGPA_OK;
}

int32_t vgpa_qknorm_rope_bwd(const void* dq_out, const void* dk_out, const void* q_in, const void* k_in, void* dq_in, void* dk_in,
                             const int64_t* dqout_strides, const int64_t* dkout_strides, const int64_t* qin_strides,
                             const int64_t* kin_strides, const int64_t* dqin_strides, const int64_t* dkin_strides, const float* wq,
                             const float* wk, const float* rope_cos, const float* rope_sin, int64_t text_len, int64_t B, int64_t H,
                             int64_t S, int64_t head_dim, float eps, int32_t rope_mode, hipStream_t stream) {
    if (!dq_out || !dk_out || !q_in || !k_in || !dq_in || !dk_in || !wq || !wk || head_dim != 64 || B <= 0 || H <= 0 || S <= 0) return VGPA_ERR_INVALID;
    if (!qs_ok(dqout_strides) || !qs_ok(dkout_strides) || !qs_ok(qin_strides) || !qs_ok(kin_strides) || !qs_ok(dqin_strides) || !qs_ok(dkin_strides))
        return VGPA_ERR_INVALID;
    if ((rope_cos == nullptr) != (rope_sin == nullptr) || text_len < 0 || text_len > S || (rope_mode != 0 && rope_mode != 1)) return VGPA_ERR_INVALID;
    const int64_t threads = 2 * B * S * H * 8;
    if (2 * B * S * H >= ((int64_t)1 << 31) || threads / 256 >= ((int64_t)1 << 31)) return VGPA_ERR_INVALID;
    VGPA_LAUNCH(qknorm_rope_bwd_kernel, dim3((unsigned)((threads + 255) / 256)), dim3(256), 0, stream, (const bf16_t*)dq_out,
                       (const bf16_t*)dk_out, (const bf16_t*)q_in, (const bf16_t*)k_in, (bf16_t*)dq_in, (bf16_t*)dk_in, qmk(dqout_strides),
                       qmk(dkout_strides), qmk(qin_strides), qmk(kin_strides), qmk(dqin_strides), qmk(dkin_strides), wq, wk, rope_cos,
                       rope_sin, (int)text_len, (int)B, (int)H, (int)S, eps, (int)rope_mode);
    VGPA_CHECK_LAUNCH();
    return VGPA_OK;
}

}
```

### videogpa_amd/ops.py

```python
import contextlib as _contextlib
import contextvars as _contextvars
import ctypes
import os as _os

import torch

from . import _lib

_DT = {torch.float32: 0, torch.bfloat16: 1}


def _stream():
    return torch.cuda.current_stream().cuda_stream


def _req(t, dtype=None, contiguous=True):
    if not t.is_cuda:
        raise RuntimeError("videogpa_amd ops need GPU tensors (no CPU fallback)")
    if dtype is not None and t.dtype != dtype:
        raise RuntimeError(f"expected {dtype}, got {t.dtype}")
    if contiguous and not t.is_contiguous():
        raise RuntimeError("expected a contiguous tensor")
    return t

# ... 613 lines not shown
    M, K = x2.shape
    q = torch.empty(M, K, dtype=torch.float8_e4m3fn, device=x2.device)
    sc = torch.empty(M, 1, dtype=torch.float32, device=x2.device)
    _timed("quant_fp8_rows", 3.0 * M * K, lambda: _lib.call("vgpa_quant_fp8_rows", x2, x2.stride(0), q, sc, M, K, _stream()), "byte")
    return q, sc


def gelu_tanh_fwd_q8(u2):
    M, K = u2.shape
    q = torch.empty(M, K, dtype=torch.float8_e4m3fn, device=u2.device)
    sc = torch.empty(M, 1, dtype=torch.float32, device=u2.device)
    _timed("gelu_tanh_fwd_q8", 3.0 * M * K, lambda: _lib.call("vgpa_gelu_tanh_fwd_q8", u2, M, K, q, sc, _stream()), "byte")
    return q, sc


def gelu_tanh_bwd_q8(u2, dy2):
    M, K = u2.shape
    q = torch.empty(M, K, dtype=torch.float8_e4m3fn, device=u2.device)
    sc = torch.empty(M, 1, dtype=torch.float32, device=u2.device)
    _timed("gelu_tanh_bwd_q8", 5.0 * M * K, lambda: _lib.call("vgpa_gelu_tanh_bwd_q8", u2, dy2, M, K, q, sc, _stream()), "byte")
    return q, sc


class Fp8Weight:

    def __init__(self, W):
        self.version = W._version
        self.q, self.s = self._rows(W.detach())
        self.qt, self.st = self._rows(W.detach().t().contiguous())

    @staticmethod
    def _rows(w):
        fmax = torch.finfo(torch.float8_e4m3fn).max
        amax = w.float().abs().amax(dim=1, keepdim=True)
        sc = torch.where(amax > 0, amax / fmax, torch.ones_like(amax))
        return (w.float() / sc).clamp(-fmax, fmax).to(torch.float8_e4m3fn), sc.t().contiguous()

    @staticmethod
    def of(W):
        c = getattr(W, "_vgpa_fp8", None)
        if c is None or c.version != W._version or c.q.device != W.device:
            c = Fp8Weight(W)
            W._vgpa_fp8 = c
        return c


def _fp8_gemm(xq, sx, wq, sw, bias=None):
    M, N, K = xq.shape[0], wq.shape[0], xq.shape[1]
    out = []

    _timed("hipblaslt_gemm_fp8 (vendor)", 2.0 * M * N * K,
           lambda: out.append(torch._scaled_mm(xq, wq.t(), scale_a=sx, scale_b=sw, bias=bias, out_dtype=torch.bfloat16)))
    return out[0]


class _Fp8FrozenLinearFn(torch.autograd.Function):
    @staticmethod
    def forward(ctx, x, W, bias):
        w8 = Fp8Weight.of(W)
        x2 = x.reshape(-1, x.shape[-1])
        if x2.stride(1) != 1:
            x2 = x2.contiguous()
        xq, sx = quant_fp8_rows(x2)
        ctx.w8 = w8
        return _fp8_gemm(xq, sx, w8.q, w8.s, bias).view(*x.shape[:-1], W.shape[0])

    @staticmethod
    def backward(ctx, dy):
        w8 = ctx.w8
        dy2 = dy.reshape(-1, dy.shape[-1])
        if dy2.stride(1) != 1:
            dy2 = dy2.contiguous()
        dq, sd = quant_fp8_rows(dy2)
        return _fp8_gemm(dq, sd, w8.qt, w8.st).view(*dy.shape[:-1], w8.qt.shape[0]), None, None


def frozen_linear_fp8(x, W, bias):
    if W.requires_grad or (bias is not None and bias.requires_grad):
        raise RuntimeError("videogpa_amd: the fp8 path is for frozen projections only")
    if x.dtype != torch.bfloat16:
        raise TypeError("frozen_linear_fp8: bf16 activations")
    return _Fp8FrozenLinearFn.apply(x, W, bias)


class _FfnTailFp8Fn(torch.autograd.Function):

    @staticmethod
    def forward(ctx, x, a, gates1, ln_w, ln_b, mod2, W1, b1, W2, b2, gates2, nxt_w, nxt_b, nxt_mod, nxt_eps, text_len, eps, n_pad, dy_pad):
        _req(x, torch.bfloat16), _req(a, torch.bfloat16), _req(gates1, torch.float32), _req(gates2, torch.float32)
        _req(ln_w, torch.float32), _req(ln_b, torch.float32), _req(nxt_w, torch.float32), _req(nxt_b, torch.float32)
        B, S, D = x.shape
        rows, dev = B * S, x.device
        keep = any(ctx.needs_input_grad)
        w1, w2 = Fp8Weight.of(W1), Fp8Weight.of(W2)
        x1 = torch.empty_like(x)
        hq = torch.empty(rows, D, dtype=torch.float8_e4m3fn, device=dev)
        hs = torch.empty(rows, 1, dtype=torch.float32, device=dev)
        mean1 = torch.empty(B, S, dtype=torch.float32, device=dev) if keep else None
        rstd1 = torch.empty_like(mean1) if keep else None
        sv, s1v, st, s1t, mstride = _mod_ptrs(mod2)
        _timed("residual_ln_fwd_fp8", 7.0 * rows * D,
               lambda: _lib.call("vgpa_residual_ln_fwd_q8", x, a, gates1[:, 0], gates1[:, 1], gates1.stride(0), ln_w, ln_b, sv, s1v, st, s1t, mstride,
                                 B, S, D, text_len, float(eps), x1, hq, hs, mean1, rstd1, _stream()), "byte")
        u = _fp8_gemm(hq, hs, w1.q, w1.s, b1)
        del hq, hs
        gq, gs = gelu_tanh_fwd_q8(u)
        f = _fp8_gemm(gq, gs, w2.q, w2.s, b2)
        del gq, gs
        x2 = torch.empty_like(x)
        n = _padded_empty((B, S), D, n_pad, x.dtype, dev) if n_pad else _empty_rows(x.shape, x.dtype, dev)
        mean2 = torch.empty(B, S, dtype=torch.float32, device=dev) if keep else None
        rstd2 = torch.empty_like(mean2) if keep else None
        nv, n1v, nt, n1t, nstride = _mod_ptrs(nxt_mod)
        _timed("residual_ln_fwd", 8.0 * rows * D,
               lambda: _lib.call("vgpa_residual_ln_fwd", x1, f, gates2[:, 0], gates2[:, 1], gates2.stride(0), nxt_w, nxt_b, nv, n1v, nt, n1t, nstride,
                                 B, S, D, text_len, float(nxt_eps), x2, n, D + n_pad, mean2, rstd2, _stream()), "byte")
        if keep:
            ctx.save_for_backward(x1, mean1, rstd1, u, x2, mean2, rstd2, ln_w, mod2, gates1, nxt_w, nxt_mod, gates2)
            ctx.w, ctx.text_len, ctx.dy_pad = (w1, w2), text_len, dy_pad
        return x2, n

    @staticmethod
    def backward(ctx, dx2, dn):
        x1, mean1, rstd1, u, x2, mean2, rstd2, ln_w, mod2, gates1, nxt_w, nxt_mod, gates2 = ctx.saved_tensors
        w1, w2 = ctx.w
        B, S, D = x1.shape
        rows, dev = B * S, x1.device
        dn = torch.zeros_like(x2) if dn is None else dn.contiguous()
        dres = None if dx2 is None else dx2.contiguous()
        dx1 = torch.empty_like(x1)
        dfq = torch.empty(rows, D, dtype=torch.float8_e4m3fn, device=dev)
        dfs = torch.empty(rows, 1, dtype=torch.float32, device=dev)
        _, n1v, _, n1t, nstride = _mod_ptrs(nxt_mod)
        _timed("residual_ln_bwd_fp8", (7.0 + (2.0 if dres is not None else 0.0)) * rows * D,
               lambda: _lib.call("vgpa_residual_ln_bwd_q8", dn, x2, mean2, rstd2, nxt_w, n1v, n1t, nstride, gates2[:, 0], gates2[:, 1], gates2.stride(0),
                                 dres, B, S, D, ctx.text_len, dx1, dfq, dfs, _stream()), "byte")
        dg = _fp8_gemm(dfq, dfs, w2.qt, w2.st)
        del dfq, dfs
        duq, dus = gelu_tanh_bwd_q8(u, dg)
        del dg
        dh = _fp8_gemm(duq, dus, w1.qt, w1.st)
        del duq, dus
        dx = torch.empty_like(x1)
        dyp = ctx.dy_pad
        da = _padded_empty((B, S), D, dyp, x1.dtype, dev) if dyp else _empty_rows(x1.shape, x1.dtype, dev)
        _, s1v, _, s1t, mstride = _mod_ptrs(mod2)
        _timed("residual_ln_bwd", 10.0 * rows * D,
               lambda: _lib.call("vgpa_residual_ln_bwd", dh, x1, mean1, rstd1, ln_w, s1v, s1t, mstride, gates1[:, 0], gates1[:, 1], gates1.stride(0),
                                 dx1, B, S, D, ctx.text_len, dx, da, D + dyp, _stream()), "byte")
        return (dx, da) + (None,) * 17


def ffn_tail_fp8(x, a, gates1, ln_w, ln_b, mod2, W1, b1, W2, b2, gates2, nxt_w, nxt_b, nxt_mod=None, nxt_eps=1e-5, text_len=0, eps=1e-5, n_pad=0, dy_pad=0):
    if W1.requires_grad or W2.requires_grad or (b1 is not None and b1.requires_grad) or (b2 is not None and b2.requires_grad):
        raise RuntimeError("videogpa_amd: the fp8 path is for frozen projections only")
    if W1.shape[0] > 16384:
        raise RuntimeError(f"ffn_tail_fp8: the GELU -> e4m3 kernels hold one feed-forward row per workgroup, inner <= 16384; got {W1.shape[0]}")
    return _FfnTailFp8Fn.apply(x, a, gates1, ln_w, ln_b, mod2, W1, b1, W2, b2, gates2, nxt_w, nxt_b, nxt_mod, nxt_eps, int(text_len), eps, int(n_pad),
                               int(dy_pad))


class _LinearLoraExtFn(torch.autograd.Function):

    @staticmethod
    def forward(ctx, x, bias, ext, enabled, scalings, x_recompute, *AB):
        K, R, N = ext.K, ext.R, ext.N
        x2 = x.reshape(-1, K)
        M = x2.shape[0]
        x_ext = _padded_base(x2, K + R)
        if x_ext is None:
            x_ext = torch.zeros(M, K + R, dtype=x.dtype, device=x.device) if not enabled else torch.empty(M, K + R, dtype=x.dtype, device=x.device)
            x_ext[:, :K].copy_(x2)
        xv, tv = x_ext[:, :K], x_ext[:, K:]
        if enabled:
            lora_down(xv, ext.A_cat, out=tv)
        ctx.rows_per_call = current_gemm_rows()
        y = _gemm(x_ext, ext.W_ext, bias, ext=True, split=ctx.rows_per_call)
        if x_recompute is not None and enabled:
            fn, srcs = x_recompute
            ctx.save_for_backward(tv.contiguous(), *srcs)
            ctx.x_fn = fn
        else:
            ctx.save_for_backward(x_ext)
            ctx.x_fn = None
        ctx.ext, ctx.enabled, ctx.xshape, ctx.scalings = ext, enabled, x.shape, scalings
        return y.view(*x.shape[:-1], N)

    @staticmethod
    def backward(ctx, dy):
        ext, enabled = ctx.ext, ctx.enabled
        saved, *srcs = ctx.saved_tensors
        K, R, N, Dn, rp, r, act = ext.K, ext.R, ext.N, ext.Dn, ext.rp, ext.r, ext.act
        dy2 = dy.reshape(-1, N)
        M = dy2.shape[0]
        dy_ext = _padded_base(dy2, N + R) if dy2.stride(1) == 1 else None
        if dy_ext is None:
            dy_ext = torch.zeros(M, N + R, dtype=dy.dtype, device=dy.device) if not enabled else torch.empty(M, N + R, dtype=dy.dtype, device=dy.device)
            dy_ext[:, :N].copy_(dy2)
        if enabled:
            for j, i in enumerate(act):
                lora_down(dy_ext[:, i * Dn:(i + 1) * Dn], ext.sBt[j], out=dy_ext[:, N + j * rp:N + (j + 1) * rp])
        dx = _gemm(dy_ext, ext.Wt_ext, ext=True, split=ctx.rows_per_call)
        out_grads = [None] * len(ctx.needs_input_grad[6:])
        if enabled:
            if ctx.x_fn is not None:
                t_all, xh = saved, ctx.x_fn(*srcs).reshape(M, K)
            else:
                t_all, xh = saved[:, K:], saved[:, :K]
            for j, i in enumerate(act):
                out_grads[2 * i + 1] = lora_grad(dy_ext[:, i * Dn:(i + 1) * Dn], t_all[:, j * rp:(j + 1) * rp], ctx.scalings[j])[:, :r]
            dA = lora_grad(dy_ext[:, N:], xh)
            for j, i in enumerate(act):
                out_grads[2 * i] = dA[j * rp:j * rp + r]
        return (dx.view(ctx.xshape), None, None, None, None, None, *out_grads)


def linear_lora_ext(x, W, bias, ext, loras, enabled=True, x_recompute=None):
    if W.requires_grad or (bias is not None and bias.requires_grad):
        raise RuntimeError("videogpa_amd: base weights are frozen on this path (LoRA-only training, as in the reference)")
    ext.refresh(W, len(loras), loras)
    flat = []
    for l in loras:
        flat += [None, None] if l is None else [l[0], l[1]]
    return _LinearLoraExtFn.apply(x, bias, ext, bool(enabled), tuple(float(loras[i][2]) for i in ext.act), x_recompute, *flat)


def linear_lora(x, W, bias, loras, ext=None):
    if all(l is None for l in loras):
        return frozen_linear(x, W, bias)
    if ext is None:
        ext = getattr(W, "_vgpa_lora_ext", None)
        if ext is None:
            ext = LoraExt()
            W._vgpa_lora_ext = ext
    return linear_lora_ext(x, W, bias, ext, loras, True)


def _bhs_strides(t):
    assert t.stride(3) == 1
    return _i64x3(t.stride(0), t.stride(1), t.stride(2))


LOG2E = 1.4426950408889634
ATTN_SPLIT_MODE = -1
def precise_delta_default():
    v = _os.environ.get("VGPA_PRECISE_DELTA", "int8").lower()
    if v in ("0", "off", "none", "false"):
        return None
    if v in ("1", "int8", "res8", "true"):
        return "int8"
    if v == "bf16":
        return "bf16"
    raise ValueError(f"VGPA_PRECISE_DELTA={v!r}: expected 0 | off | int8 | bf16")


def _res_kind(o_res):
    if o_res is None:
        return 0
    if o_res.dtype == torch.bfloat16:
        return 1
    if o_res.dtype == torch.uint8:
        return 2
    raise TypeError(f"o_res: bf16 (rounding residual) or uint8 (eight further mantissa bits), got {o_res.dtype}")


def res8_decode(o, o_res8):
    E = (o.contiguous().view(torch.int16).to(torch.int32) >> 7) & 0xFF
    sc = torch.where(E > 15, torch.ldexp(torch.ones((), device=o.device), E - 142), torch.zeros((), device=o.device))
    return o.float() + (o_res8.float() - 128.0) * sc


def prescale_q(q, scale=None):
    scale = q.shape[-1] ** -0.5 if scale is None else scale
    return (q.float() * (scale * LOG2E)).to(q.dtype)


class AttnFwdPolicy:
    SWITCH, CHECKS, RECHECK = 0.5, 2, 1024

    def __init__(self, mode="bound", fixed=False):
        self.mode, self.fixed = mode, fixed
        self.calls = 0
        self.redo_fraction = None
        self.switched_at = None

    def wants_flags(self):
        return self.mode == "bound" and not self.fixed and (self.calls < self.CHECKS or self.calls % self.RECHECK == 0)

    def observe(self, fraction):
        self.redo_fraction = fraction
        if not self.fixed and fraction > self.SWITCH:
            self.mode, self.switched_at = "online", self.calls


def _strip_flags(ws, head_words, B, H, Sq):
    strips = (Sq + 255) // 256
    return ws[:4 * (head_words + B * H * strips)].view(torch.int32)[head_words:].view(B, H, strips)


def attention_redo_fraction(ws, B, H, S):
    return float((_strip_flags(ws, B * H, B, H, S) != 0).float().mean())


def attention_fwd_raw(q, k, v, scale=None, q_prescaled=False, split_mode=None, o_pad=0, o_res=None, policy=None):
    B, H, S, Dh = q.shape
    scale = Dh ** -0.5 if scale is None else scale
    if not q_prescaled:
        q = prescale_q(q, scale)
    o = _padded_empty((B, S), H * Dh, o_pad, torch.bfloat16, q.device) if o_pad else torch.empty(B, S, H * Dh, dtype=torch.bfloat16, device=q.device)
    lse = torch.empty(B, H, S, dtype=torch.float32, device=q.device)
    ov = o.unflatten(-1, (H, Dh)).permute(0, 2, 1, 3)
    split_mode = ATTN_SPLIT_MODE if split_mode is None else split_mode
    ws_bytes = _lib.query("vgpa_attn_fwd_w1_workspace_bytes", B, H, S)
    ws = torch.empty(ws_bytes, dtype=torch.uint8, device=q.device)
    rv = None if o_res is None else o_res.unflatten(-1, (H, Dh)).permute(0, 2, 1, 3)
    entry = "vgpa_attn_fwd_online_res" if (policy is not None and policy.mode == "online") else "vgpa_attn_fwd_w1_res"
    _timed("attn_fwd_kernel", 4.0 * S * S * Dh * B * H, lambda: _lib.call(
        entry, q, k, v, o, o_res, _res_kind(o_res), lse, _bhs_strides(q), _bhs_strides(k), _bhs_strides(v), _bhs_strides(ov), None if rv is None else _bhs_strides(rv),
        B, H, S, Dh, float(scale), int(split_mode), ws, ws_bytes, _stream()))
    if policy is not None:
        if policy.wants_flags() and not torch.cuda.is_current_stream_capturing():
            policy.observe(attention_redo_fraction(ws, B, H, S))
        policy.calls += 1
    return o, lse


def attention_bwd_raw(q, k, v, o, do, lse, dq, dk, dv, scale=None, q_prescaled=False, split_mode=None, o_res=None):
    B, H, S, Dh = q.shape
    scale = Dh ** -0.5 if scale is None else scale
    if not q_prescaled:
        q = prescale_q(q, scale)
    delta = torch.empty(B, H, S, dtype=torch.float32, device=q.device)
    st = _stream()
    stats = torch.empty(B, H, 2, S, dtype=torch.float32, device=q.device)
    _timed("attn_delta_kernel", (4.0 + (0 if o_res is None else o_res.element_size())) * B * H * S * Dh, lambda: _lib.call(
        "vgpa_attn_bwd_prep_w1_res", o, o_res, _res_kind(o_res), do, lse, _bhs_strides(o), None if o_res is None else _bhs_strides(o_res), _bhs_strides(do),
        delta, stats, B, H, S, Dh, st), "byte")
    split_mode = ATTN_SPLIT_MODE if split_mode is None else split_mode
    ws_bytes = _lib.query("vgpa_attn_bwd_split_workspace_bytes", B, H, S) if split_mode != 0 else 0
    ws = torch.empty(max(ws_bytes, 16), dtype=torch.uint8, device=q.device)
    wsp = ws if ws_bytes else None
    _timed("attn_bwd_dkv_kernel", 6.0 * S * S * Dh * B * H, lambda: _lib.call(
        "vgpa_attn_bwd_dkv_w1", q, k, v, do, stats, dk, dv, _bhs_strides(q), _bhs_strides(k), _bhs_strides(v), _bhs_strides(do),
        _bhs_strides(dk), _bhs_strides(dv), B, H, S, Dh, float(scale), int(split_mode), wsp, ws_bytes, st))
    _timed("attn_bwd_dq_kernel", 2.0 * S * S * Dh * B * H, lambda: _lib.call(
        "vgpa_attn_bwd_dq_w1", q, k, v, do, lse, delta, dq, _bhs_strides(q), _bhs_strides(k), _bhs_strides(v), _bhs_strides(do),
        _bhs_strides(dq), B, H, S, Dh, float(scale), int(split_mode), wsp, ws_bytes, st))


ATTN128_W1 = True


ATTN128_F8_MIN_KEYS = 1024


def attention128_uses_f8(f8, Skv):
    return bool(f8) and Skv >= ATTN128_F8_MIN_KEYS


class F8AttnPolicy:
    ERR_PER_BOUND = 0.004

    def __init__(self, mode="f8", fixed=False, threshold=0.5):
        self.mode, self.fixed, self.threshold = mode, fixed, float(threshold)
        self.decided = False
        self.estimated_score_error = None

    def reset(self):
        self.decided = False

    @staticmethod
    def score_error_estimate(q, k, H, scale):
        B, Lq, D = q.shape
        d = D // H
        qn = q.view(B, Lq, H, d).float().pow(2).sum(-1).amax(dim=1).sqrt()
        kn = k.view(B, k.shape[1], H, d).float().pow(2).sum(-1).amax(dim=1).sqrt()
        return float((qn * kn).amax()) * float(scale) * LOG2E * F8AttnPolicy.ERR_PER_BOUND

    def use_f8(self, q, k, H, scale):
        if not self.fixed and not self.decided and self.mode == "f8":
            self.estimated_score_error = self.score_error_estimate(q, k, H, scale)
            if self.estimated_score_error > self.threshold:
                self.mode = "bf16"
        self.decided = True
        return self.mode == "f8"


def attention128_f8_redo_fraction(ws, B, H, Sq):
    return float((_strip_flags(ws, 5 * B * H, B, H, Sq) != 0).float().mean())


def attention128_fwd_raw(q, k, v, scale, o_pad=0, f8=False, o_res8=None, deq=None, report=None):
    B, H, Sq, D = q.shape
    Skv = k.shape[2]
    assert D == 128 and k.shape == (B, H, Skv, 128) and v.shape == k.shape and q.dtype == k.dtype == v.dtype == torch.bfloat16
    o2 = _padded_empty((B, Sq), H * D, o_pad, torch.bfloat16, q.device) if o_pad else torch.empty(B, Sq, H * D, dtype=torch.bfloat16, device=q.device)
    o = o2.unflatten(-1, (H, D)).permute(0, 2, 1, 3)
    lse = torch.empty(B, H, Sq, dtype=torch.float32, device=q.device)
    rv = rs = None
    if o_res8 is not None:
        if o_res8.dtype != torch.uint8 or o_res8.shape != (B, Sq, H * D) or not o_res8.is_contiguous():
            raise TypeError("attention128_fwd_raw: o_res8 is a contiguous uint8 [B, Sq, H*128] buffer")
        rv = o_res8.unflatten(-1, (H, D)).permute(0, 2, 1, 3)
        rs = _bhs_strides(rv)
    if attention128_uses_f8(f8, Skv):
        ws_bytes = _lib.query("vgpa_attn128_fwd_f8_workspace_bytes", B, H, Sq, Skv)
        ws = torch.empty(ws_bytes, dtype=torch.uint8, device=q.device)
        dv_ = [None] * 3
        if deq is not None:
            for t, S_ in zip(deq, (Sq, Skv, Skv)):
                if t.dtype != torch.bfloat16 or t.shape != (B, S_, H * D) or not t.is_contiguous():
                    raise TypeError("attention128_fwd_raw: deq = three contiguous bf16 [B, S, H*128] buffers (q, k, v)")
            dv_ = [t.unflatten(-1, (H, D)).permute(0, 2, 1, 3) for t in deq]
        ds_ = [None if t is None else _bhs_strides(t) for t in dv_]
        _timed("attn128_fwd_f8", 4.0 * B * H * Sq * Skv * D, lambda: _lib.call(
            "vgpa_attn128_fwd_f8", q, k, v, o, lse, _bhs_strides(q), _bhs_strides(k), _bhs_strides(v), _bhs_strides(o), rv, rs, dv_[0], dv_[1], dv_[2],
            ds_[0], ds_[1], ds_[2], B, H, Sq, Skv, float(scale), ws, ws_bytes, _stream()))
        if report is not None:
            report["redo_fraction"] = attention128_f8_redo_fraction(ws, B, H, Sq)
            report["strip_flags"] = _strip_flags(ws, 5 * B * H, B, H, Sq) != 0
        return o, lse
    if deq is not None:
        raise ValueError("attention128_fwd_raw: deq buffers are written by the e4m3 forward only (f8=True and at least ATTN128_F8_MIN_KEYS keys)")
    ws_bytes = _lib.query("vgpa_attn128_fwd_workspace_bytes", B, H, Sq) if ATTN128_W1 else 0
    ws = torch.empty(ws_bytes, dtype=torch.uint8, device=q.device) if ws_bytes else None
    _timed("attn128_fwd" if Skv >= 1024 else "attn128_fwd (short keys)", 4.0 * B * H * Sq * Skv * D, lambda: _lib.call(
        "vgpa_attn128_fwd", q, k, v, o, lse, _bhs_strides(q), _bhs_strides(k), _bhs_strides(v), _bhs_strides(o), rv, rs, B, H, Sq, Skv, float(scale),
        ws, ws_bytes, _stream()))
    return o, lse


def attention128_bwd_raw(q, k, v, o, do, lse, dq, dk, dv, scale, o_res8=None, q_prescaled=False):
    B, H, Sq, D = q.shape
    Skv = k.shape[2]
    rv = None if o_res8 is None else o_res8.unflatten(-1, (H, D)).permute(0, 2, 1, 3)
    ws_bytes = _lib.query("vgpa_attn128_bwd_workspace_bytes", B, H, Sq)
    ws = torch.empty(ws_bytes, dtype=torch.uint8, device=q.device)
    _timed("attn128_bwd" if Skv >= 1024 else "attn128_bwd (short keys)", 8.0 * B * H * Sq * Skv * D, lambda: _lib.call(
        "vgpa_attn128_bwd_prescaled" if q_prescaled else "vgpa_attn128_bwd", q, k, v, o, do, lse, dq, dk, dv, _bhs_strides(q), _bhs_strides(k), _bhs_strides(v), _bhs_strides(o), _bhs_strides(do),
        _bhs_strides(dq), _bhs_strides(dk), _bhs_strides(dv), rv, None if rv is None else _bhs_strides(rv), B, H, Sq, Skv, float(scale),
        -1 if ATTN128_W1 else 0, ws, ws_bytes, _stream()))


class _Attention128Fn(torch.autograd.Function):

    @staticmethod
    def forward(ctx, q, k, v, scale, o_pad, precise_delta):
        q, k, v = (t if t.stride(3) == 1 else t.contiguous() for t in (q, k, v))
        o_res8 = None
        if precise_delta and any(ctx.needs_input_grad[:3]):
            o_res8 = torch.empty(q.shape[0], q.shape[2], q.shape[1] * q.shape[3], dtype=torch.uint8, device=q.device)
        o, lse = attention128_fwd_raw(q, k, v, scale, o_pad, o_res8=o_res8)
        ctx.save_for_backward(q, k, v, o, lse, o_res8)
        ctx.scale = float(scale)
        return o

    @staticmethod
    def backward(ctx, do):
        q, k, v, o, lse, o_res8 = ctx.saved_tensors
        B, H, Sq, D = q.shape
        Skv = k.shape[2]
        do = do if do.stride(3) == 1 else do.contiguous()
        dq = torch.empty(B, Sq, H, D, dtype=torch.bfloat16, device=q.device).permute(0, 2, 1, 3)
        dk = torch.empty(B, Skv, H, D, dtype=torch.bfloat16, device=q.device).permute(0, 2, 1, 3)
        dv = torch.empty(B, Skv, H, D, dtype=torch.bfloat16, device=q.device).permute(0, 2, 1, 3)
        attention128_bwd_raw(q, k, v, o, do, lse, dq, dk, dv, ctx.scale, o_res8=o_res8)
        return dq, dk, dv, None, None, None


def attention128(q, k, v, scale=None, o_pad=0, precise_delta="int8"):
    if precise_delta not in (None, "int8"):
        raise ValueError('attention128: precise_delta is "int8" or None (the bf16 residual form exists at head_dim 64 only)')
    return _Attention128Fn.apply(q, k, v, q.shape[-1] ** -0.5 if scale is None else scale, int(o_pad), precise_delta)


class _QKNormAttentionFn(torch.autograd.Function):

    @staticmethod
    def forward(ctx, qkv, wq, bq, wk, bk, rope_cos, rope_sin, text_len, H, eps, o_pad, grad_pad, rope_mode=0, recompute_qk=False, precise_delta=None, fwd_policy=None):
        _req(qkv, torch.bfloat16)
        B, S, W = qkv.shape
        Dh = W // (3 * H)
        qkv5 = qkv.view(B, S, 3, H, Dh)
        q_in, k_in, v = (qkv5[:, :, i].permute(0, 2, 1, 3) for i in range(3))
        qn = torch.empty(B, H, S, Dh, dtype=torch.bfloat16, device=qkv.device)
        kn = torch.empty_like(qn)
        _timed("qknorm_rope_fwd", 8.0 * B * H * S * Dh, lambda: _lib.call(
            "vgpa_qknorm_rope_fwd", q_in, k_in, qn, kn, _bhs_strides(q_in), _bhs_strides(k_in), _bhs_strides(qn), _bhs_strides(kn),
            wq, bq, wk, bk, rope_cos, rope_sin, text_len, B, H, S, Dh, float(eps), float(Dh ** -0.5 * LOG2E), int(rope_mode), _stream()), "byte")
        o_res = None
        if precise_delta and ctx.needs_input_grad[0]:
            o_res = torch.empty(B, S, H * Dh, dtype=torch.uint8 if precise_delta == "int8" else torch.bfloat16, device=qkv.device)
        o, lse = attention_fwd_raw(qn, kn, v, q_prescaled=True, o_pad=o_pad, o_res=o_res, policy=fwd_policy)
        if recompute_qk:
            ctx.save_for_backward(qkv, o, lse, wq, wk, rope_cos, rope_sin, bq, bk, o_res)
        else:
            ctx.save_for_backward(qkv, qn, kn, o, lse, wq, wk, rope_cos, rope_sin, o_res)
        ctx.meta = (text_len, H, eps, grad_pad, int(rope_mode), bool(recompute_qk))
        return o

    @staticmethod
    def backward(ctx, do):
        text_len, H, eps, grad_pad, rope_mode, recompute_qk = ctx.meta
        if recompute_qk:
            qkv, o, lse, wq, wk, rope_cos, rope_sin, bq, bk, o_res = ctx.saved_tensors
        else:
            qkv, qn, kn, o, lse, wq, wk, rope_cos, rope_sin, o_res = ctx.saved_tensors
        B, S, W = qkv.shape
        Dh = W // (3 * H)
        do = do.contiguous()
        qkv5 = qkv.view(B, S, 3, H, Dh)
        q_in, k_in, v = (qkv5[:, :, i].permute(0, 2, 1, 3) for i in range(3))
        if recompute_qk:
            qn = torch.empty(B, H, S, Dh, dtype=torch.bfloat16, device=qkv.device)
            kn = torch.empty_like(qn)
            _timed("qknorm_rope_fwd", 8.0 * B * H * S * Dh, lambda: _lib.call(
                "vgpa_qknorm_rope_fwd", q_in, k_in, qn, kn, _bhs_strides(q_in), _bhs_strides(k_in), _bhs_strides(qn), _bhs_strides(kn),
                wq, bq, wk, bk, rope_cos, rope_sin, text_len, B, H, S, Dh, float(eps), float(Dh ** -0.5 * LOG2E), int(rope_mode), _stream()), "byte")
        dqkv = _padded_empty((B, S), W, grad_pad, qkv.dtype, qkv.device) if grad_pad else torch.empty_like(qkv)
        d5 = dqkv.unflatten(-1, (3, H, Dh))
        dq_in, dk_in, dv = (d5[:, :, i].permute(0, 2, 1, 3) for i in range(3))
        dqn = torch.empty_like(qn)
        dkn = torch.empty_like(kn)
        ov = o.unflatten(-1, (H, Dh)).permute(0, 2, 1, 3)
        dov = do.view(B, S, H, Dh).permute(0, 2, 1, 3)
        attention_bwd_raw(qn, kn, v, ov, dov, lse, dqn, dkn, dv, q_prescaled=True,
                          o_res=None if o_res is None else o_res.unflatten(-1, (H, Dh)).permute(0, 2, 1, 3))
        _timed("qknorm_rope_bwd", 12.0 * B * H * S * Dh, lambda: _lib.call(
            "vgpa_qknorm_rope_bwd", dqn, dkn, q_in, k_in, dq_in, dk_in, _bhs_strides(dqn), _bhs_strides(dkn), _bhs_strides(q_in),
            _bhs_strides(k_in), _bhs_strides(dq_in), _bhs_strides(dk_in), wq, wk, rope_cos, rope_sin, text_len, B, H, S, Dh,
            float(eps), rope_mode, _stream()), "byte")
        return dqkv, None, None, None, None, None, None, None, None, None, None, None, None, None, None, None


def qknorm_attention(qkv, wq, bq, wk, bk, H, text_len=0, rope=None, eps=1e-6, o_pad=0, grad_pad=0, rope_mode=0, recompute_qk=False, precise_delta="int8", fwd_policy=None):
    cos, sin = (None, None) if rope is None else rope
    if precise_delta not in (None, "int8", "bf16"):
        raise ValueError(f'precise_delta: "int8", "bf16" or None, got {precise_delta!r}')
    return _QKNormAttentionFn.apply(qkv, wq, bq, wk, bk, cos, sin, text_len, H, eps, o_pad, grad_pad, rope_mode, bool(recompute_qk), precise_delta, fwd_policy)


def rope2d_tables(pos, head_dim=64, frequency=100.0):
    half = head_dim // 2
    inv = 1.0 / (frequency ** (torch.arange(0, half, 2, device=pos.device).float() / half))
    ang = pos.float()[:, :, None] * inv[None, None, :]
    ang = torch.cat([ang, ang], dim=-1).reshape(pos.shape[0], head_dim)
    return ang.cos().contiguous(), ang.sin().contiguous()


def _heads_in(*ts):
    for t in ts:
        if t is None:
            continue
        _req(t, torch.float32)
        if torch.is_grad_enabled() and t.requires_grad:
            raise RuntimeError("the fp32 head kernels are forward only: call them under torch.no_grad()")


def pack_conv_weight(w):
    return w.detach().float().permute(2, 3, 1, 0).contiguous()


def conv3x3_f32(x, w_packed, bias=None, res=None, res2=None, relu_in=False, relu_res=False, stride=1):
    _heads_in(x, w_packed, bias, res, res2)
    N, H, W, Cin = x.shape
    Cout = w_packed.shape[-1]
    if tuple(w_packed.shape) != (3, 3, Cin, Cout) or Cin % 16 or Cout % 16:
        raise RuntimeError(f"conv3x3_f32: weight {tuple(w_packed.shape)} does not fit input channels {Cin} (multiples of 16)")
    Ho, Wo = (H - 1) // stride + 1, (W - 1) // stride + 1
    out = torch.empty(N, Ho, Wo, Cout, device=x.device, dtype=torch.float32)
    for r in (res, res2):
        if r is not None and r.shape != out.shape:
            raise RuntimeError("conv3x3_f32: residual shape differs from the output's")
    _timed("conv3x3_f32", 2.0 * out.numel() * 9 * Cin,
           lambda: _lib.call("vgpa_conv3x3_f32", x, w_packed, bias, res, res2, out, N, H, W, Cin, Cout, stride,
                             (1 if relu_in else 0) | (2 if relu_res else 0), _stream()))
    return out


def conv1x1_f32(x, w_packed, bias=None):
    _heads_in(x, w_packed, bias)
    Cin, Cout = w_packed.shape
    if x.shape[-1] != Cin or Cin % 16 or Cout % 16:
        raise RuntimeError(f"conv1x1_f32: weight {tuple(w_packed.shape)} does not fit input {tuple(x.shape)} (channels in multiples of 16)")
    out = torch.empty(*x.shape[:-1], Cout, device=x.device, dtype=torch.float32)
    M = out.numel() // Cout
    _timed("conv1x1_f32", 2.0 * M * Cin * Cout, lambda: _lib.call("vgpa_conv1x1_f32", x, w_packed, bias, out, M, Cin, Cout, _stream()))
    return out


def uv_embed_tables(width, height, channels, aspect_ratio, device, ratio=0.1, f32_angles=False):
    if channels % 8:
        raise RuntimeError("uv_embed_tables: channels must be a multiple of 8")
    diag = (aspect_ratio ** 2 + 1.0) ** 0.5
    span_x, span_y = aspect_ratio / diag, 1.0 / diag
    xs = torch.linspace(-span_x * (width - 1) / width, span_x * (width - 1) / width, steps=width, dtype=torch.float32)
    ys = torch.linspace(-span_y * (height - 1) / height, span_y * (height - 1) / height, steps=height, dtype=torch.float32)
    half = channels // 2
    adt = torch.float32 if f32_angles else torch.float64
    omega = torch.arange(half // 2, dtype=adt)
    omega /= half / 2.0
    omega = 1.0 / 100 ** omega

    def table(pos):
        ang = torch.einsum("m,d->md", pos.to(adt), omega)
        return (torch.cat([ang.sin(), ang.cos()], dim=1).float() * ratio).contiguous().to(device)
    return table(xs), table(ys)


def upsample_bilinear_ac_f32(x, H, W, tabs=None):
    xt, yt = tabs if tabs is not None else (None, None)
    _heads_in(x, xt, yt)
    N, h, w, C = x.shape
    if xt is not None and (tuple(xt.shape) != (W, C // 2) or tuple(yt.shape) != (H, C // 2)):
        raise RuntimeError("upsample_bilinear_ac_f32: embedding tables do not fit the output")
    out = torch.empty(N, H, W, C, device=x.device, dtype=torch.float32)
    _timed("upsample_bilinear_ac_f32", 4.0 * out.numel(), lambda: _lib.call("vgpa_upsample_bilinear_ac_f32", x, xt, yt, out, N, h, w, C, H, W, _stream()),
           unit="byte")
    return out


_DPT_ACT = {"exp": 0, "inv_log": 1}


def _tail_fits(name, x, H, W, w1_packed, w2, xt, yt, grid):
    C, od = x.shape[3], w2.shape[0]
    if tuple(w1_packed.shape) != (3, 3, C, 32) or tuple(w2.shape) != (od, 32) or C % 16:
        raise RuntimeError(f"{name}: weights do not fit the input")
    if xt is not None and (tuple(xt.shape) != (W, C // 2) or tuple(yt.shape) != (H, C // 2)):
        raise RuntimeError(f"{name}: embedding tables do not fit the {grid}")


def dpt_tail_f32(x, H, W, w1_packed, b1, w2, b2, activation="exp", tabs=None):
    xt, yt = tabs if tabs is not None else (None, None)
    _heads_in(x, xt, yt, w1_packed, b1, w2, b2)
    if activation not in _DPT_ACT:
        raise NotImplementedError(f"dpt_tail_f32: activation {activation!r} (exp and inv_log are built)")
    N, h, w, C = x.shape
    od = w2.shape[0]
    _tail_fits("dpt_tail_f32", x, H, W, w1_packed, w2, xt, yt, "output")
    preds = torch.empty(N, H, W, od - 1, device=x.device, dtype=torch.float32)
    conf = torch.empty(N, H, W, device=x.device, dtype=torch.float32)
    _timed("dpt_tail_f32", 2.0 * N * H * W * (9 * C * 32 + 32 * od),
           lambda: _lib.call("vgpa_dpt_tail_f32", x, xt, yt, w1_packed, b1, w2, b2, preds, conf, N, h, w, C, H, W, od, _DPT_ACT[activation], _stream()))
    return preds, conf


def dualdpt_aux_tail_f32(x, w1_packed, b1, ln_w, ln_b, eps, w2, b2, tabs=None):
    xt, yt = tabs if tabs is not None else (None, None)
    _heads_in(x, xt, yt, w1_packed, b1, ln_w, ln_b, w2, b2)
    N, h, w, C = x.shape
    od = w2.shape[0]
    if not 2 <= od <= 8:
        raise RuntimeError("dualdpt_aux_tail_f32: weights do not fit the input")
    _tail_fits("dualdpt_aux_tail_f32", x, h, w, w1_packed, w2, xt, yt, "map")
    if b1.numel() != 32 or ln_w.numel() != 32 or ln_b.numel() != 32 or b2.numel() != od:
        raise RuntimeError("dualdpt_aux_tail_f32: biases / LayerNorm parameters do not fit 32 hidden channels and the output width")
    preds = torch.empty(N, h, w, od - 1, device=x.device, dtype=torch.float32)
    conf = torch.empty(N, h, w, device=x.device, dtype=torch.float32)
    _timed("dualdpt_aux_tail_f32", 2.0 * N * h * w * (9 * C * 32 + 32 * od),
           lambda: _lib.call("vgpa_dualdpt_aux_tail_f32", x, xt, yt, w1_packed, b1, ln_w, ln_b, float(eps), w2, b2, preds, conf, N, h, w, C, od, _stream()))
    return preds, conf


def attn_small_f32(qkv, scale=None):
    _heads_in(qkv)
    B, S, three, H, D = qkv.shape
    if three != 3 or S > 128 or D % 32 or D > 256:
        raise RuntimeError(f"attn_small_f32: qkv {tuple(qkv.shape)} outside S <= 128, D in multiples of 32 up to 256")
    o = torch.empty(B, S, H * D, device=qkv.device, dtype=torch.float32)
    q, k, v = qkv[:, :, 0], qkv[:, :, 1], qkv[:, :, 2]
    _timed("attn_small_f32", 4.0 * B * H * S * S * D,
           lambda: _lib.call("vgpa_attn_small_f32", q, k, v, S * 3 * H * D, D, 3 * H * D, o, B, H, S, D, float(scale if scale is not None else D ** -0.5),
                             _stream()))
    return o


def pack_patch_weight(conv_weight):
    C = conv_weight.shape[0]
    w = conv_weight.detach().float().reshape(C, -1).t()
    K = w.shape[0]
    out = torch.zeros((K + 15) // 16 * 16, C, device=w.device, dtype=torch.float32)
    out[:K] = w
    return out


def dino_embed(images, w_packed, bias, cls, reg, pos, out_dtype=torch.bfloat16):
    _req(images)
    for t in (w_packed, bias, cls, reg, pos):
        if t is not None:
            _req(t, torch.float32)
    if torch.is_grad_enabled() and any(t is not None and t.requires_grad for t in (images, w_packed, bias, cls, reg, pos)):
        raise RuntimeError("dino_embed is forward only: call it under torch.no_grad()")
    if images.dtype not in _DT or out_dtype not in _DT:
        raise RuntimeError(f"dino_embed: fp32 or bf16 images and output, got {images.dtype} -> {out_dtype}")
    N, three, H, W = images.shape
    Kpad, C = w_packed.shape
    if three != 3 or (Kpad // 3) < 1:
        raise RuntimeError(f"dino_embed: images {tuple(images.shape)} are not [N,3,H,W]")
    R = 0 if reg is None else reg.shape[-2]
    cls, pos = cls.reshape(-1), pos.reshape(-1, C)
    reg = None if reg is None else reg.reshape(R, C)
    p = next((c for c in range(1, 65) if (3 * c * c + 15) // 16 * 16 == Kpad and H % c == 0 and pos.shape[0] == 1 + (H // c) * (W // c)), None) \
        if W > 0 and H > 0 else None
    if p is None or W % p or bias.numel() != C or cls.numel() != C or C % 32:
        raise RuntimeError(f"dino_embed: weight {tuple(w_packed.shape)}, position table {tuple(pos.shape)} and images {tuple(images.shape)} do not "
                           "fit one patch size (H, W multiples of it; channels a multiple of 32)")
    P = (H // p) * (W // p)
    out = torch.empty(N, 1 + R + P, C, device=images.device, dtype=out_dtype)
    _timed("dino_embed", 2.0 * N * P * C * 3 * p * p,
           lambda: _lib.call("vgpa_dino_embed", images, _DT[images.dtype], w_packed, Kpad, bias, cls, reg, pos, out, _DT[out_dtype], N, H, W, p, C, R,
                             _stream()))
    return out


def stream_ln(x, y=None, gamma=None, ln_w=None, ln_b=None, eps=1e-6, n_dtype=torch.bfloat16):
    _req(x, torch.float32)
    for t, dt in ((y, torch.bfloat16), (gamma, torch.float32), (ln_w, torch.float32), (ln_b, torch.float32)):
        if t is not None:
            _req(t, dt)
    if torch.is_grad_enabled() and any(t is not None and t.requires_grad for t in (x, y, gamma, ln_w, ln_b)):
        raise RuntimeError("stream_ln is forward only: call it under torch.no_grad()")
    D = x.shape[-1]
    if (y is not None and y.shape != x.shape) or any(t is not None and t.numel() != D for t in (gamma, ln_w, ln_b)) or n_dtype not in _DT:
        raise RuntimeError("stream_ln: shapes of x, y, gamma and the LayerNorm parameters do not fit")
    x_new = torch.empty_like(x) if y is not None else None
    n = torch.empty(x.shape, device=x.device, dtype=n_dtype) if ln_w is not None else None
    M = x.numel() // D
    nbytes = 4.0 + (6.0 if y is not None else 0.0) + (0.0 if n is None else n.element_size())
    _timed("stream_ln_f32", nbytes * M * D,
           lambda: _lib.call("vgpa_stream_ln_f32", x, y, gamma, ln_w, ln_b, x_new, n, _DT[n_dtype], M, D, float(eps), _stream()), "byte")
    return x_new, n


LPIPS_SHIFT = (-.030, -.088, -.188)
LPIPS_SCALE = (.458, .448, .450)


def lpips_input_f32(x, shift=LPIPS_SHIFT, scale=LPIPS_SCALE, normalize=False, out=None):
    _heads_in(x, out)
    if x.dim() != 4 or x.shape[1] != 3:
        raise RuntimeError(f"lpips_input_f32: expected [N,3,H,W], got {tuple(x.shape)}")
    N, _, H, W = x.shape
    if out is None:
        out = torch.empty(N, H, W, 16, device=x.device, dtype=torch.float32)
    elif tuple(out.shape) != (N, H, W, 16):
        raise RuntimeError("lpips_input_f32: `out` must be [N,H,W,16]")
    _timed("lpips_input_f32", 4.0 * (x.numel() + out.numel()),
           lambda: _lib.call("vgpa_lpips_input_f32", x, out, N, H, W, *[float(v) for v in shift], *[float(v) for v in scale], 1 if normalize else 0,
                             _stream()), "byte")
    return out


def maxpool2x2_f32(x, relu=False):
    _heads_in(x)
    N, H, W, C = x.shape
    if H < 2 or W < 2 or C % 4:
        raise RuntimeError(f"maxpool2x2_f32: needs H, W >= 2 and channels in multiples of 4, got {tuple(x.shape)}")
    out = torch.empty(N, H // 2, W // 2, C, device=x.device, dtype=torch.float32)
    _timed("maxpool2x2_f32", 4.0 * (4 * out.numel() + out.numel()),
           lambda: _lib.call("vgpa_maxpool2x2_f32", x, out, N, H, W, C, 1 if relu else 0, _stream()), "byte")
    return out


def lpips_layer_f32(f0, f1, w, relu=False, total=None, accumulate=False, out=None):
    _heads_in(f0, f1, w, out)
    N, H, W, C = f0.shape
    if f1.shape != f0.shape or w.numel() != C or C % 4 or C > 512:
        raise RuntimeError(f"lpips_layer_f32: maps {tuple(f0.shape)} / {tuple(f1.shape)} and weight {tuple(w.shape)} do not fit (C % 4 == 0, C <= 512)")
    if total is not None:
        _req(total, torch.float64)
        if total.numel() != N:
            raise RuntimeError("lpips_layer_f32: `total` must hold N values")
    if out is None:
        out = torch.empty(N, device=f0.device, dtype=torch.float32)
    elif out.numel() != N:
        raise RuntimeError("lpips_layer_f32: `out` must hold N values")
    ws_bytes = _lib.query("vgpa_lpips_layer_workspace_bytes", N, H, W, C)
    ws = torch.empty(ws_bytes, dtype=torch.uint8, device=f0.device)
    _timed("lpips_layer_f32", 2.0 * f0.numel() * 4,
           lambda: _lib.call("vgpa_lpips_layer_f32", f0, f1, w, out, total, N, H, W, C, (1 if relu else 0) | (2 if accumulate else 0), ws, ws_bytes,
                             _stream()), "byte")
    return out


def _dtype_code(dtype, name):
    if dtype not in (torch.float32, torch.bfloat16):
        raise RuntimeError(f"{name}: float32 or bfloat16, got {dtype}")
    return 1 if dtype == torch.bfloat16 else 0


def conv3x3_pad_f32(x, w_packed, bias=None, res=None, stride=1, pad_lo=1, pad_hi=1):
    _heads_in(x, w_packed, bias, res)
    N, H, W, Cin = x.shape
    Cout = w_packed.shape[-1]
    if tuple(w_packed.shape) != (3, 3, Cin, Cout) or Cin % 16 or Cout % 16:
# ... 193 lines not shown
```

Baseline: 0.4452 pair-steps/s.

## Fuse attention delta prep into dQ kernel and k-max into qknorm-rope

```diff
diff --git a/include/videogpa_hip.h b/include/videogpa_hip.h
--- a/include/videogpa_hip.h
+++ b/include/videogpa_hip.h
@@ -71,6 +71,11 @@
                              const float* wq, const float* bq, const float* wk, const float* bk, const float* rope_cos,
                              const float* rope_sin, int64_t text_len, int64_t B, int64_t H, int64_t S, int64_t head_dim,
                              float eps, float q_out_scale, int32_t rope_mode, vgpa_stream_t stream);
+int32_t vgpa_qknorm_rope_fwd_kmax(const void* q_in, const void* k_in, void* q_out, void* k_out, const int64_t* qin_strides,
+                                  const int64_t* kin_strides, const int64_t* qout_strides, const int64_t* kout_strides,
+                                  const float* wq, const float* bq, const float* wk, const float* bk, const float* rope_cos,
+                                  const float* rope_sin, int64_t text_len, int64_t B, int64_t H, int64_t S, int64_t head_dim,
+                                  float eps, float q_out_scale, int32_t rope_mode, void* kmax2, vgpa_stream_t stream);
 int32_t vgpa_qknorm_rope_bwd(const void* dq_out, const void* dk_out, const void* q_in, const void* k_in, void* dq_in,
                              void* dk_in, const int64_t* dqout_strides, const int64_t* dkout_strides,
                              const int64_t* qin_strides, const int64_t* kin_strides, const int64_t* dqin_strides,
@@ -94,6 +99,10 @@
                              const int64_t* k_strides, const int64_t* v_strides, const int64_t* o_strides, const int64_t* ores_strides,
                              int64_t B, int64_t H, int64_t S, int64_t head_dim, float scale, int32_t split_mode, void* workspace,
                              size_t ws_bytes, vgpa_stream_t stream);
+int32_t vgpa_attn_fwd_w1_kmax(const void* q, const void* k, const void* v, void* o, void* o_res, int32_t res_kind, float* lse2, const int64_t* q_strides,
+                              const int64_t* k_strides, const int64_t* v_strides, const int64_t* o_strides, const int64_t* ores_strides,
+                              int64_t B, int64_t H, int64_t S, int64_t head_dim, float scale, int32_t split_mode, void* workspace,
+                              size_t ws_bytes, vgpa_stream_t stream);
 int32_t vgpa_attn_fwd_online_res(const void* q, const void* k, const void* v, void* o, void* o_res, int32_t res_kind, float* lse2, const int64_t* q_strides,
                                  const int64_t* k_strides, const int64_t* v_strides, const int64_t* o_strides, const int64_t* ores_strides,
                                  int64_t B, int64_t H, int64_t S, int64_t head_dim, float scale, int32_t split_mode, void* workspace,
@@ -101,6 +110,11 @@
 int32_t vgpa_attn_bwd_prep_w1_res(const void* o, const void* o_res, int32_t res_kind, const void* d_o, const float* lse2, const int64_t* o_strides,
                                   const int64_t* ores_strides, const int64_t* do_strides, float* delta, float* stats, int64_t B, int64_t H,
                                   int64_t S, int64_t head_dim, vgpa_stream_t stream);
+int32_t vgpa_attn_bwd_dq_stats_w1(const void* q, const void* k, const void* v, const void* d_o, const void* o, const void* o_res, int32_t res_kind,
+                                  const float* lse2, float* delta, float* stats, void* dq, const int64_t* q_strides, const int64_t* k_strides,
+                                  const int64_t* v_strides, const int64_t* do_strides, const int64_t* o_strides, const int64_t* ores_strides,
+                                  const int64_t* dq_strides, int64_t B, int64_t H, int64_t S, int64_t head_dim, float scale, int32_t split_mode,
+                                  void* workspace, size_t ws_bytes, vgpa_stream_t stream);
 int32_t vgpa_attn_bwd_dkv_w1(const void* q, const void* k, const void* v, const void* d_o, const float* stats, void* dk, void* dv,
                              const int64_t* q_strides, const int64_t* k_strides, const int64_t* v_strides, const int64_t* do_strides,
                              const int64_t* dk_strides, const int64_t* dv_strides, int64_t B, int64_t H, int64_t S, int64_t head_dim,
diff --git a/videogpa_amd/_lib.py b/videogpa_amd/_lib.py
--- a/videogpa_amd/_lib.py
+++ b/videogpa_amd/_lib.py
@@ -26,6 +26,7 @@
     "vgpa_gelu_tanh_fwd": (I32, [P, I64, P, P]),
     "vgpa_gelu_tanh_bwd": (I32, [P, P, I64, P, P]),
     "vgpa_qknorm_rope_fwd": (I32, [P, P, P, P, P, P, P, P, P, P, P, P, P, P, I64, I64, I64, I64, I64, F32, F32, I32, P]),
+    "vgpa_qknorm_rope_fwd_kmax": (I32, [P, P, P, P, P, P, P, P, P, P, P, P, P, P, I64, I64, I64, I64, I64, F32, F32, I32, P, P]),
     "vgpa_qknorm_rope_bwd": (I32, [P, P, P, P, P, P, P, P, P, P, P, P, P, P, P, P, I64, I64, I64, I64, I64, F32, I32, P]),
     "vgpa_grad_norm_workspace_bytes": (SZ, []),
     "vgpa_grad_norm": (I32, [P, I64, F32, P, P, SZ, P]),
@@ -35,7 +36,9 @@
     "vgpa_attn_fwd_w1_workspace_bytes": (SZ, [I64, I64, I64]),
     "vgpa_attn_bwd_prep_w1_res": (I32, [P, P, I32, P, P, P, P, P, P, P, I64, I64, I64, I64, P]),
     "vgpa_attn_fwd_w1_res": (I32, [P, P, P, P, P, I32, P, P, P, P, P, P, I64, I64, I64, I64, F32, I32, P, SZ, P]),
+    "vgpa_attn_fwd_w1_kmax": (I32, [P, P, P, P, P, I32, P, P, P, P, P, P, I64, I64, I64, I64, F32, I32, P, SZ, P]),
     "vgpa_attn_fwd_online_res": (I32, [P, P, P, P, P, I32, P, P, P, P, P, P, I64, I64, I64, I64, F32, I32, P, SZ, P]),
+    "vgpa_attn_bwd_dq_stats_w1": (I32, [P, P, P, P, P, P, I32, P, P, P, P, P, P, P, P, P, P, P, I64, I64, I64, I64, F32, I32, P, SZ, P]),
     "vgpa_attn_bwd_dkv_w1": (I32, [P, P, P, P, P, P, P, P, P, P, P, P, P, I64, I64, I64, I64, F32, I32, P, SZ, P]),
     "vgpa_attn_bwd_split_workspace_bytes": (SZ, [I64, I64, I64]),
     "vgpa_lora_down": (I32, [P, I64, P, P, I64, I64, I64, I64, P]),
diff --git a/videogpa_amd/csrc/attention_w1.hip b/videogpa_amd/csrc/attention_w1.hip
--- a/videogpa_amd/csrc/attention_w1.hip
+++ b/videogpa_amd/csrc/attention_w1.hip
@@ -11,7 +11,9 @@
                                                                   const float* __restrict__ LSE2, const float* __restrict__ DELTA,
                                                                   bf16_t* __restrict__ dQ, TStride sq, TStride sk, TStride sv, TStride sdo,
                                                                   TStride sdq, int S, int H, int n_qt, float scale, int task0, int nsplit,
-                                                                  float* __restrict__ part) {
+                                                                  float* __restrict__ part, const bf16_t* __restrict__ O,
+                                                                  const void* __restrict__ ORES, TStride so, TStride sor, int res_kind,
+                                                                  float* __restrict__ STATS, float* __restrict__ DELTA_OUT) {
     constexpr int QB = 2;
     __shared__ __attribute__((aligned(1024))) uint8_t lds[W1_RING_BYTES];
     int vid, chunk;
@@ -28,14 +30,72 @@
     for (int j = 0; j < QB; ++j) {
         load_row_frags(Q + ((size_t)b * sq.b + (size_t)h * sq.h), sq.s, q0 + 32 * j, S, lane, qf[j]);
         load_row_frags(dO + ((size_t)b * sdo.b + (size_t)h * sdo.h), sdo.s, q0 + 32 * j, S, lane, dof[j]);
-        int qc = q0 + 32 * j + (lane & 31);
-        qc = qc < S ? qc : S - 1;
-        const float nl = -LSE2[(int64_t)bh * S + qc], nd = -DELTA[(int64_t)bh * S + qc];
-#pragma unroll
-        for (int i = 0; i < 16; ++i) { cs[j][i] = nl; cd[j][i] = nd; }
+    }
+    float nl[QB];
+    u32x4_t ob[QB][4], rb[QB][4];
+#pragma unroll
+    for (int j = 0; j < QB; ++j) {
+        const int q = q0 + 32 * j + (lane & 31);
+        const int qc = q < S ? q : S - 1;
+        nl[j] = -LSE2[(int64_t)bh * S + qc];
+        if (O) {
+            const bf16_t* Op = O + ((size_t)b * so.b + (size_t)h * so.h + (size_t)qc * so.s + (size_t)(hi * 8));
+            const size_t ro = (size_t)b * sor.b + (size_t)h * sor.h + (size_t)qc * sor.s + (size_t)(hi * 8);
+#pragma unroll
+            for (int ks = 0; ks < 4; ++ks) {
+                ob[j][ks] = *reinterpret_cast<const u32x4_t*>(Op + ks * 16);
+                if (res_kind == VGPA_RES_8) {
+                    const u32x2_t r2 = *reinterpret_cast<const u32x2_t*>((const uint8_t*)ORES + ro + ks * 16);
+                    rb[j][ks][0] = r2[0]; rb[j][ks][1] = r2[1];
+                } else if (res_kind == VGPA_RES_BF16) {
+                    rb[j][ks] = *reinterpret_cast<const u32x4_t*>((const bf16_t*)ORES + ro + ks * 16);
+                }
+            }
+        }
     }
 #pragma unroll
     for (int j = 0; j < QB; ++j) { frags_arrived(qf[j]); frags_arrived(dof[j]); }
+#pragma unroll
+    for (int j = 0; j < QB; ++j) {
+        const int q = q0 + 32 * j + (lane & 31);
+        const int qc = q < S ? q : S - 1;
+        float nd;
+        if (O) {
+            float g[4];
+#pragma unroll
+            for (int ks = 0; ks < 4; ++ks) {
+                float a[8], o[8];
+                unpack8(__builtin_bit_cast(u32x4_t, dof[j][ks]), a);
+                if (res_kind == VGPA_RES_8) {
+                    const u32x2_t r2 = {rb[j][ks][0], rb[j][ks][1]};
+                    unpack8_res8(ob[j][ks], r2, o);
+                } else {
+                    unpack8(ob[j][ks], o);
+                    if (res_kind == VGPA_RES_BF16) {
+                        float r[8];
+                        unpack8(rb[j][ks], r);
+#pragma unroll
+                        for (int i = 0; i < 8; ++i) o[i] += r[i];
+                    }
+                }
+                float acc = 0.f;
+#pragma unroll
+                for (int i = 0; i < 8; ++i) acc += a[i] * o[i];
+                g[ks] = acc + other_half(acc);
+            }
+            const float d = (g[0] + g[1]) + (g[2] + g[3]);
+            nd = -d;
+            if (hi == 0 && q < S && (!SPLIT || chunk == 0)) {
+                STATS[(int64_t)bh * 2 * S + q] = nl[j];
+                STATS[(int64_t)bh * 2 * S + S + q] = nd;
+                if (DELTA_OUT) DELTA_OUT[(int64_t)bh * S + q] = d;
+            }
+        } else {
+            nd = -DELTA[(int64_t)bh * S + qc];
+        }
+#pragma unroll
+        for (int i = 0; i < 16; ++i) { cs[j][i] = nl[j]; cd[j][i] = nd; }
+    }
 
     const W1Range tr = w1_split_range(S, chunk, nsplit, SPLIT);
     const int tb = tr.tb, nt = tr.nt;
@@ -510,14 +570,20 @@
     return (size_t)max_split_parts(tasks, W1_MAX_SPLIT, w1_slots()) * part * sizeof(float);
 }
 
-int32_t vgpa_attn_bwd_dq_w1(const void* q, const void* k, const void* v, const void* d_o, const float* lse2, const float* delta, void* dq,
-                            const int64_t* q_strides, const int64_t* k_strides, const int64_t* v_strides, const int64_t* do_strides,
-                            const int64_t* dq_strides, int64_t B, int64_t H, int64_t S, int64_t head_dim, float scale, int32_t split_mode,
-                            void* workspace, size_t ws_bytes, hipStream_t stream) {
-    if (!q || !k || !v || !d_o || !lse2 || !delta || !dq || head_dim != HD || B <= 0 || H <= 0 || S <= 0 || S > (1 << 24)) return VGPA_ERR_INVALID;
+static int32_t bwd_dq_w1_impl(const void* q, const void* k, const void* v, const void* d_o, const float* lse2, const float* delta_in, void* dq,
+                              const int64_t* q_strides, const int64_t* k_strides, const int64_t* v_strides, const int64_t* do_strides,
+                              const int64_t* dq_strides, int64_t B, int64_t H, int64_t S, int64_t head_dim, float scale, int32_t split_mode,
+                              void* workspace, size_t ws_bytes, hipStream_t stream, const void* o, const void* o_res, int32_t res_kind,
+                              const int64_t* o_strides, const int64_t* ores_strides, float* stats, float* delta_out) {
+    if (!q || !k || !v || !d_o || !lse2 || !dq || head_dim != HD || B <= 0 || H <= 0 || S <= 0 || S > (1 << 24)) return VGPA_ERR_INVALID;
+    if (o ? !stats : !delta_in) return VGPA_ERR_INVALID;
     if (!view_ok(q_strides, B, H, S, HD) || !view_ok(k_strides, B, H, S, HD) || !view_ok(v_strides, B, H, S, HD) || !view_ok(do_strides, B, H, S, HD) ||
         !view_ok(dq_strides, B, H, S, HD) || !al16(q) || !al16(k) || !al16(v) || !al16(d_o) || !al16(dq) || (workspace && !al16(workspace)))
         return VGPA_ERR_INVALID;
+    if (o && (!view_ok(o_strides, B, H, S, HD) || !al16(o))) return VGPA_ERR_INVALID;
+    if (o && o_res && (!view_ok(ores_strides, B, H, S, HD) || !al16(o_res) || (res_kind != VGPA_RES_BF16 && res_kind != VGPA_RES_8))) return VGPA_ERR_INVALID;
+    const int rk = (o && o_res) ? (int)res_kind : VGPA_RES_NONE;
+    const TStride so = o ? mk(o_strides) : mk(do_strides), sor = (o && o_res) ? mk(ores_strides) : so;
     const int rows = 256;
     W1Plan pl;
     const int32_t rc = plan_w1(B, H, S, split_mode, W1_MAX_SPLIT, w1_slots(), W1_DQ_PART_FLOATS * sizeof(float), workspace, ws_bytes, 0, &pl);
@@ -526,20 +592,38 @@
     const TailSplit& p = pl.p;
     if (p.n_main > 0) {
         VGPA_LAUNCH((attn_bwd_dq_w1_kernel<false>), dim3((unsigned)p.n_main), dim3(256), 0, stream, (const bf16_t*)q, (const bf16_t*)k,
-                    (const bf16_t*)v, (const bf16_t*)d_o, lse2, delta, (bf16_t*)dq, mk(q_strides), mk(k_strides), mk(v_strides), mk(do_strides),
-                    mk(dq_strides), (int)S, (int)H, n_t, scale, 0, 1, (float*)nullptr);
+                    (const bf16_t*)v, (const bf16_t*)d_o, lse2, delta_in, (bf16_t*)dq, mk(q_strides), mk(k_strides), mk(v_strides), mk(do_strides),
+                    mk(dq_strides), (int)S, (int)H, n_t, scale, 0, 1, (float*)nullptr, (const bf16_t*)o, o_res, so, sor, rk, stats, delta_out);
         VGPA_CHECK_LAUNCH();
     }
     if (p.n_tail > 0) {
         VGPA_LAUNCH((attn_bwd_dq_w1_kernel<true>), dim3((unsigned)(p.n_tail * p.nsplit)), dim3(256), 0, stream, (const bf16_t*)q, (const bf16_t*)k,
-                    (const bf16_t*)v, (const bf16_t*)d_o, lse2, delta, (bf16_t*)dq, mk(q_strides), mk(k_strides), mk(v_strides), mk(do_strides),
-                    mk(dq_strides), (int)S, (int)H, n_t, scale, (int)p.n_main, p.nsplit, (float*)workspace);
+                    (const bf16_t*)v, (const bf16_t*)d_o, lse2, delta_in, (bf16_t*)dq, mk(q_strides), mk(k_strides), mk(v_strides), mk(do_strides),
+                    mk(dq_strides), (int)S, (int)H, n_t, scale, (int)p.n_main, p.nsplit, (float*)workspace, (const bf16_t*)o, o_res, so, sor, rk, stats,
+                    delta_out);
         VGPA_CHECK_LAUNCH();
         VGPA_LAUNCH(w1_dq_merge_kernel, dim3((unsigned)(p.n_tail * (rows / 4))), dim3(256), 0, stream, (const float*)workspace, p.nsplit, (int)p.n_main, n_t,
                     rows, (bf16_t*)dq, mk(dq_strides), (int)S, (int)H, scale);
         VGPA_CHECK_LAUNCH();
     }
     return VGPA_OK;
+}
+int32_t vgpa_attn_bwd_dq_w1(const void* q, const void* k, const void* v, const void* d_o, const float* lse2, const float* delta, void* dq,
+                            const int64_t* q_strides, const int64_t* k_strides, const int64_t* v_strides, const int64_t* do_strides,
+                            const int64_t* dq_strides, int64_t B, int64_t H, int64_t S, int64_t head_dim, float scale, int32_t split_mode,
+                            void* workspace, size_t ws_bytes, hipStream_t stream) {
+    if (!delta) return VGPA_ERR_INVALID;
+    return bwd_dq_w1_impl(q, k, v, d_o, lse2, delta, dq, q_strides, k_strides, v_strides, do_strides, dq_strides, B, H, S, head_dim, scale, split_mode, workspace,
+                          ws_bytes, stream, nullptr, nullptr, VGPA_RES_NONE, nullptr, nullptr, nullptr, nullptr);
+}
+int32_t vgpa_attn_bwd_dq_stats_w1(const void* q, const void* k, const void* v, const void* d_o, const void* o, const void* o_res, int32_t res_kind,
+                                  const float* lse2, float* delta, float* stats, void* dq, const int64_t* q_strides, const int64_t* k_strides,
+                                  const int64_t* v_strides, const int64_t* do_strides, const int64_t* o_strides, const int64_t* ores_strides,
+                                  const int64_t* dq_strides, int64_t B, int64_t H, int64_t S, int64_t head_dim, float scale, int32_t split_mode,
+                                  void* workspace, size_t ws_bytes, hipStream_t stream) {
+    if (!o || !stats) return VGPA_ERR_INVALID;
+    return bwd_dq_w1_impl(q, k, v, d_o, lse2, nullptr, dq, q_strides, k_strides, v_strides, do_strides, dq_strides, B, H, S, head_dim, scale, split_mode, workspace,
+                          ws_bytes, stream, o, o_res, res_kind, o_strides, ores_strides, stats, delta);
 }
 
 
@@ -600,7 +684,7 @@
 static int32_t fwd_w1_impl(const void* q, const void* k, const void* v, void* o, void* o_res, int32_t res_kind, float* lse2, const int64_t* q_strides,
                            const int64_t* k_strides, const int64_t* v_strides, const int64_t* o_strides, const int64_t* ores_strides, int64_t B,
                            int64_t H, int64_t S, int64_t head_dim, float scale, int32_t split_mode, void* workspace, size_t ws_bytes,
-                           hipStream_t stream, bool force_online) {
+                           hipStream_t stream, bool force_online, bool kmax_valid) {
     (void)scale;
     if (!q || !k || !v || !o || !lse2 || !workspace || head_dim != HD || B <= 0 || H <= 0 || S <= 0 || S > (1 << 24)) return VGPA_ERR_INVALID;
     if (!view_ok(q_strides, B, H, S, HD) || !view_ok(k_strides, B, H, S, HD) || !view_ok(v_strides, B, H, S, HD) || !view_ok(o_strides, B, H, S, HD) ||
@@ -627,9 +711,13 @@
         return vgpa_internal_attn_fwd_redo(q, k, v, o, lse2, mk(q_strides), mk(k_strides), mk(v_strides), mk(o_strides), (int)S, (int)H, n_qt, tasks,
                                            flags, stream, ores, sor, rk);
     }
-    if (hipMemsetAsync(workspace, 0, head, stream) != hipSuccess) return VGPA_ERR_LAUNCH;
-    VGPA_LAUNCH((w1_kmax_kernel<HD / 8>), dim3(16, (unsigned)(B * H)), dim3(256), 0, stream, (const bf16_t*)k, mk(k_strides), (int)S, (int)H, kmax2);
-    VGPA_CHECK_LAUNCH();
+    if (kmax_valid) {
+        if (hipMemsetAsync(flags, 0, head - (size_t)(B * H) * 4, stream) != hipSuccess) return VGPA_ERR_LAUNCH;
+    } else {
+        if (hipMemsetAsync(workspace, 0, head, stream) != hipSuccess) return VGPA_ERR_LAUNCH;
+        VGPA_LAUNCH((w1_kmax_kernel<HD / 8>), dim3(16, (unsigned)(B * H)), dim3(256), 0, stream, (const bf16_t*)k, mk(k_strides), (int)S, (int)H, kmax2);
+        VGPA_CHECK_LAUNCH();
+    }
     if (p.n_main > 0) {
         VGPA_LAUNCH((attn_fwd_w1_kernel<false>), dim3((unsigned)p.n_main), dim3(256), 0, stream, (const bf16_t*)q, (const bf16_t*)k, (const bf16_t*)v,
                     (bf16_t*)o, lse2, (const unsigned*)kmax2, flags, mk(q_strides), mk(k_strides), mk(v_strides), mk(o_strides), (int)S, (int)H, n_qt, 0, 1,
@@ -653,14 +741,21 @@
                              int64_t H, int64_t S, int64_t head_dim, float scale, int32_t split_mode, void* workspace, size_t ws_bytes,
                              hipStream_t stream) {
     return fwd_w1_impl(q, k, v, o, o_res, res_kind, lse2, q_strides, k_strides, v_strides, o_strides, ores_strides, B, H, S, head_dim, scale, split_mode, workspace,
-                       ws_bytes, stream, false);
+                       ws_bytes, stream, false, false);
+}
+int32_t vgpa_attn_fwd_w1_kmax(const void* q, const void* k, const void* v, void* o, void* o_res, int32_t res_kind, float* lse2, const int64_t* q_strides,
+                              const int64_t* k_strides, const int64_t* v_strides, const int64_t* o_strides, const int64_t* ores_strides, int64_t B,
+                              int64_t H, int64_t S, int64_t head_dim, float scale, int32_t split_mode, void* workspace, size_t ws_bytes,
+                              hipStream_t stream) {
+    return fwd_w1_impl(q, k, v, o, o_res, res_kind, lse2, q_strides, k_strides, v_strides, o_strides, ores_strides, B, H, S, head_dim, scale, split_mode, workspace,
+                       ws_bytes, stream, false, true);
 }
 int32_t vgpa_attn_fwd_online_res(const void* q, const void* k, const void* v, void* o, void* o_res, int32_t res_kind, float* lse2, const int64_t* q_strides,
                                  const int64_t* k_strides, const int64_t* v_strides, const int64_t* o_strides, const int64_t* ores_strides, int64_t B,
                                  int64_t H, int64_t S, int64_t head_dim, float scale, int32_t split_mode, void* workspace, size_t ws_bytes,
                                  hipStream_t stream) {
     return fwd_w1_impl(q, k, v, o, o_res, res_kind, lse2, q_strides, k_strides, v_strides, o_strides, ores_strides, B, H, S, head_dim, scale, split_mode, workspace,
-                       ws_bytes, stream, true);
-}
-
-}
+                       ws_bytes, stream, true, false);
+}
+
+}
diff --git a/videogpa_amd/csrc/qknorm.hip b/videogpa_amd/csrc/qknorm.hip
--- a/videogpa_amd/csrc/qknorm.hip
+++ b/videogpa_amd/csrc/qknorm.hip
@@ -7,6 +7,65 @@
     v += __shfl_xor(v, 2, 64);
     v += __shfl_xor(v, 4, 64);
     return v;
+}
+
+template <bool KMAX>
+__device__ __forceinline__ float qknorm_rope_fwd_row(const bf16_t* __restrict__ q_in, const bf16_t* __restrict__ k_in, bf16_t* __restrict__ q_out,
+                                                     bf16_t* __restrict__ k_out, const QStride& si_q, const QStride& si_k, const QStride& so_q,
+                                                     const QStride& so_k, const float* __restrict__ wq, const float* __restrict__ bq,
+                                                     const float* __restrict__ wk, const float* __restrict__ bk, const float* __restrict__ rope_cos,
+                                                     const float* __restrict__ rope_sin, int text_len, float eps, float q_out_scale, int rope_mode,
+                                                     int which, int b, int h, int s, int c8) {
+    const bf16_t* ip = which ? (k_in + b * si_k.b + h * si_k.h + (int64_t)s * si_k.s) : (q_in + b * si_q.b + h * si_q.h + (int64_t)s * si_q.s);
+    bf16_t* op = which ? (k_out + b * so_k.b + h * so_k.h + (int64_t)s * so_k.s) : (q_out + b * so_q.b + h * so_q.h + (int64_t)s * so_q.s);
+    const float* w = which ? wk : wq;
+    const float* bb = which ? bk : bq;
+    float x[8];
+    unpack8(*reinterpret_cast<const u32x4_t*>(ip + c8 * 8), x);
+    float sum = 0.f;
+#pragma unroll
+    for (int j = 0; j < 8; ++j) sum += x[j];
+    const float mean = group8_sum(sum) * (1.f / 64.f);
+    float sq = 0.f;
+#pragma unroll
+    for (int j = 0; j < 8; ++j) { const float d = x[j] - mean; sq += d * d; }
+    const float rstd = rsqrtf(group8_sum(sq) * (1.f / 64.f) + eps);
+    float y[8];
+#pragma unroll
+    for (int j = 0; j < 8; ++j) y[j] = (x[j] - mean) * rstd * w[c8 * 8 + j] + bb[c8 * 8 + j];
+    if (rope_cos && rope_mode == 1) {
+        const bool on = s >= text_len;
+        const float* cp = rope_cos + (int64_t)(on ? s - text_len : 0) * 64 + c8 * 8;
+        const float* sp = rope_sin + (int64_t)(on ? s - text_len : 0) * 64 + c8 * 8;
+        const float sgn = (c8 & 2) ? 1.f : -1.f;
+#pragma unroll
+        for (int j = 0; j < 8; ++j) {
+            const float partner = __shfl_xor(y[j], 2, 64);
+            if (on) y[j] = y[j] * cp[j] + sgn * partner * sp[j];
+        }
+    } else if (rope_cos && s >= text_len) {
+        const float* cp = rope_cos + (int64_t)(s - text_len) * 64 + c8 * 8;
+        const float* sp = rope_sin + (int64_t)(s - text_len) * 64 + c8 * 8;
+#pragma unroll
+        for (int j = 0; j < 8; j += 2) {
+            const float a = y[j], bq2 = y[j + 1];
+            y[j] = a * cp[j] - bq2 * sp[j];
+            y[j + 1] = bq2 * cp[j + 1] + a * sp[j + 1];
+        }
+    }
+    if (!which) {
+#pragma unroll
+        for (int j = 0; j < 8; ++j) y[j] *= q_out_scale;
+    }
+    const u32x4_t packed = pack8(y);
+    *reinterpret_cast<u32x4_t*>(op + c8 * 8) = packed;
+    if (!KMAX) return 0.f;
+    float f[8];
+    unpack8(packed, f);
+    float a = 0.f;
+#pragma unroll
+    for (int j = 0; j < 8; ++j) a += f[j] * f[j];
+    return group8_sum(a);
 }
 
 __global__ __launch_bounds__(256) void qknorm_rope_fwd_kernel(const bf16_t* __restrict__ q_in, const bf16_t* __restrict__ k_in,
@@ -26,48 +85,44 @@
     const int h = (int)(r % (uint32_t)H); r /= (uint32_t)H;
     const int s = (int)(r % (uint32_t)S);
     const int b = (int)(r / (uint32_t)S);
-    const bf16_t* ip = which ? (k_in + b * si_k.b + h * si_k.h + (int64_t)s * si_k.s) : (q_in + b * si_q.b + h * si_q.h + (int64_t)s * si_q.s);
-    bf16_t* op = which ? (k_out + b * so_k.b + h * so_k.h + (int64_t)s * so_k.s) : (q_out + b * so_q.b + h * so_q.h + (int64_t)s * so_q.s);
-    const float* w = which ? wk : wq;
-    const float* bb = which ? bk : bq;
-    float x[8];
-    unpack8(*reinterpret_cast<const u32x4_t*>(ip + c8 * 8), x);
-    float sum = 0.f;
-#pragma unroll
-    for (int j = 0; j < 8; ++j) sum += x[j];
-    const float mean = group8_sum(sum) * (1.f / 64.f);
-    float sq = 0.f;
-#pragma unroll
-    for (int j = 0; j < 8; ++j) { const float d = x[j] - mean; sq += d * d; }
-    const float rstd = rsqrtf(group8_sum(sq) * (1.f / 64.f) + eps);
-    float y[8];
-#pragma unroll
-    for (int j = 0; j < 8; ++j) y[j] = (x[j] - mean) * rstd * w[c8 * 8 + j] + bb[c8 * 8 + j];
-    if (rope_cos && rope_mode == 1) {
-        const bool on = s >= text_len;
-        const float* cp = rope_cos + (int64_t)(on ? s - text_len : 0) * 64 + c8 * 8;
-        const float* sp = rope_sin + (int64_t)(on ? s - text_len : 0) * 64 + c8 * 8;
-        const float sgn = (c8 & 2) ? 1.f : -1.f;
-#pragma unroll
-        for (int j = 0; j < 8; ++j) {
-            const float partner = __shfl_xor(y[j], 2, 64);
-            if (on) y[j] = y[j] * cp[j] + sgn * partner * sp[j];
-        }
-    } else if (rope_cos && s >= text_len) {
-        const float* cp = rope_cos + (int64_t)(s - text_len) * 64 + c8 * 8;
-        const float* sp = rope_sin + (int64_t)(s - text_len) * 64 + c8 * 8;
-#pragma unroll
-        for (int j = 0; j < 8; j += 2) {
-            const float a = y[j], bq2 = y[j + 1];
-            y[j] = a * cp[j] - bq2 * sp[j];
-            y[j + 1] = bq2 * cp[j + 1] + a * sp[j + 1];
-        }
-    }
-    if (!which) {
-#pragma unroll
-        for (int j = 0; j < 8; ++j) y[j] *= q_out_scale;
-    }
-    *reinterpret_cast<u32x4_t*>(op + c8 * 8) = pack8(y);
+    (void)qknorm_rope_fwd_row<false>(q_in, k_in, q_out, k_out, si_q, si_k, so_q, so_k, wq, bq, wk, bk, rope_cos, rope_sin, text_len, eps, q_out_scale,
+                                     rope_mode, which, b, h, s, c8);
+}
+
+#define QK_TILE_TOKENS 8
+#define QK_KMAX_MAX_HEADS 256
+__global__ __launch_bounds__(256) void qknorm_rope_fwd_kmax_kernel(const bf16_t* __restrict__ q_in, const bf16_t* __restrict__ k_in,
+                                                                     bf16_t* __restrict__ q_out, bf16_t* __restrict__ k_out, QStride si_q,
+                                                                     QStride si_k, QStride so_q, QStride so_k, const float* __restrict__ wq,
+                                                                     const float* __restrict__ bq, const float* __restrict__ wk,
+                                                                     const float* __restrict__ bk, const float* __restrict__ rope_cos,
+                                                                     const float* __restrict__ rope_sin, int text_len, int B, int H, int S,
+                                                                     float eps, float q_out_scale, int rope_mode, int n_tiles ,
+                                                                     unsigned* __restrict__ kmax2) {
+    __shared__ unsigned hmax[QK_KMAX_MAX_HEADS];
+    uint32_t r = blockIdx.x;
+    const int tile = (int)(r % (uint32_t)n_tiles); r /= (uint32_t)n_tiles;
+    const int b = (int)(r % (uint32_t)B);
+    const int which = (int)(r / (uint32_t)B);
+    const int c8 = (int)threadIdx.x & 7;
+    if (which) {
+        for (int i = threadIdx.x; i < H; i += 256) hmax[i] = 0u;
+        __syncthreads();
+    }
+    const int s0 = tile * QK_TILE_TOKENS;
+    const uint32_t nv = (uint32_t)((S - s0 < QK_TILE_TOKENS ? S - s0 : QK_TILE_TOKENS) * H);
+    for (uint32_t v = threadIdx.x >> 3; v < nv; v += 32) {
+        const int h = (int)(v % (uint32_t)H), s = s0 + (int)(v / (uint32_t)H);
+        const float a = qknorm_rope_fwd_row<true>(q_in, k_in, q_out, k_out, si_q, si_k, so_q, so_k, wq, bq, wk, bk, rope_cos, rope_sin, text_len, eps,
+                                                  q_out_scale, rope_mode, which, b, h, s, c8);
+        if (which && c8 == 0 && a > 0.f) atomicMax(&hmax[h], __float_as_uint(a));
+    }
+    if (!which) return;
+    __syncthreads();
+    for (int i = threadIdx.x; i < H; i += 256) {
+        unsigned* dst = kmax2 + (b * H + i);
+        if (hmax[i] > __hip_atomic_load(dst, __ATOMIC_RELAXED, __HIP_MEMORY_SCOPE_AGENT)) atomicMax(dst, hmax[i]);
+    }
 }
 
 __global__ __launch_bounds__(256) void qknorm_rope_bwd_kernel(const bf16_t* __restrict__ dq_out, const bf16_t* __restrict__ dk_out,
@@ -143,21 +198,47 @@
 
 extern "C" {
 
+static int32_t qknorm_rope_fwd_impl(const void* q_in, const void* k_in, void* q_out, void* k_out, const int64_t* qin_strides,
+                                    const int64_t* kin_strides, const int64_t* qout_strides, const int64_t* kout_strides, const float* wq,
+                                    const float* bq, const float* wk, const float* bk, const float* rope_cos, const float* rope_sin,
+                                    int64_t text_len, int64_t B, int64_t H, int64_t S, int64_t head_dim, float eps, float q_out_scale,
+                                    int32_t rope_mode, unsigned* kmax2, hipStream_t stream) {
+    if (!q_in || !k_in || !q_out || !k_out || !wq || !bq || !wk || !bk || head_dim != 64 || B <= 0 || H <= 0 || S <= 0) return VGPA_ERR_INVALID;
+    if (!qs_ok(qin_strides) || !qs_ok(kin_strides) || !qs_ok(qout_strides) || !qs_ok(kout_strides)) return VGPA_ERR_INVALID;
+    if ((rope_cos == nullptr) != (rope_sin == nullptr) || text_len < 0 || text_len > S || (rope_mode != 0 && rope_mode != 1)) return VGPA_ERR_INVALID;
+    const int64_t threads = 2 * B * S * H * 8;
+    if (2 * B * S * H >= ((int64_t)1 << 31) || threads / 256 >= ((int64_t)1 << 31)) return VGPA_ERR_INVALID;
+    if (kmax2) {
+        const int64_t n_tiles = (S + QK_TILE_TOKENS - 1) / QK_TILE_TOKENS, blocks = 2 * B * n_tiles;
+        if (blocks >= ((int64_t)1 << 31) || H > QK_KMAX_MAX_HEADS || ((uintptr_t)kmax2 & 3)) return VGPA_ERR_INVALID;
+        if (hipMemsetAsync(kmax2, 0, (size_t)(B * H) * sizeof(unsigned), stream) != hipSuccess) return VGPA_ERR_LAUNCH;
+        VGPA_LAUNCH(qknorm_rope_fwd_kmax_kernel, dim3((unsigned)blocks), dim3(256), 0, stream, (const bf16_t*)q_in, (const bf16_t*)k_in, (bf16_t*)q_out,
+                    (bf16_t*)k_out, qmk(qin_strides), qmk(kin_strides), qmk(qout_strides), qmk(kout_strides), wq, bq, wk, bk, rope_cos, rope_sin,
+                    (int)text_len, (int)B, (int)H, (int)S, eps, q_out_scale, (int)rope_mode, (int)n_tiles, kmax2);
+        VGPA_CHECK_LAUNCH();
+        return VGPA_OK;
+    }
+    VGPA_LAUNCH(qknorm_rope_fwd_kernel, dim3((unsigned)((threads + 255) / 256)), dim3(256), 0, stream, (const bf16_t*)q_in,
+                       (const bf16_t*)k_in, (bf16_t*)q_out, (bf16_t*)k_out, qmk(qin_strides), qmk(kin_strides), qmk(qout_strides),
+                       qmk(kout_strides), wq, bq, wk, bk, rope_cos, rope_sin, (int)text_len, (int)B, (int)H, (int)S, eps, q_out_scale, (int)rope_mode);
+    VGPA_CHECK_LAUNCH();
+    return VGPA_OK;
+}
 int32_t vgpa_qknorm_rope_fwd(const void* q_in, const void* k_in, void* q_out, void* k_out, const int64_t* qin_strides,
                              const int64_t* kin_strides, const int64_t* qout_strides, const int64_t* kout_strides, const float* wq,
                              const float* bq, const float* wk, const float* bk, const float* rope_cos, const float* rope_sin,
                              int64_t text_len, int64_t B, int64_t H, int64_t S, int64_t head_dim, float eps, float q_out_scale,
                              int32_t rope_mode, hipStream_t stream) {
-    if (!q_in || !k_in || !q_out || !k_out || !wq || !bq || !wk || !bk || head_dim != 64 || B <= 0 || H <= 0 || S <= 0) return VGPA_ERR_INVALID;
-    if (!qs_ok(qin_strides) || !qs_ok(kin_strides) || !qs_ok(qout_strides) || !qs_ok(kout_strides)) return VGPA_ERR_INVALID;
-    if ((rope_cos == nullptr) != (rope_sin == nullptr) || text_len < 0 || text_len > S || (rope_mode != 0 && rope_mode != 1)) return VGPA_ERR_INVALID;
-    const int64_t threads = 2 * B * S * H * 8;
-    if (2 * B * S * H >= ((int64_t)1 << 31) || threads / 256 >= ((int64_t)1 << 31)) return VGPA_ERR_INVALID;
-    VGPA_LAUNCH(qknorm_rope_fwd_kernel, dim3((unsigned)((threads + 255) / 256)), dim3(256), 0, stream, (const bf16_t*)q_in,
-                       (const bf16_t*)k_in, (bf16_t*)q_out, (bf16_t*)k_out, qmk(qin_strides), qmk(kin_strides), qmk(qout_strides),
-                       qmk(kout_strides), wq, bq, wk, bk, rope_cos, rope_sin, (int)text_len, (int)B, (int)H, (int)S, eps, q_out_scale, (int)rope_mode);
-    VGPA_CHECK_LAUNCH();
-    return VGPA_OK;
+    return qknorm_rope_fwd_impl(q_in, k_in, q_out, k_out, qin_strides, kin_strides, qout_strides, kout_strides, wq, bq, wk, bk, rope_cos, rope_sin, text_len,
+                                B, H, S, head_dim, eps, q_out_scale, rope_mode, nullptr, stream);
+}
+int32_t vgpa_qknorm_rope_fwd_kmax(const void* q_in, const void* k_in, void* q_out, void* k_out, const int64_t* qin_strides,
+                                  const int64_t* kin_strides, const int64_t* qout_strides, const int64_t* kout_strides, const float* wq,
+                                  const float* bq, const float* wk, const float* bk, const float* rope_cos, const float* rope_sin,
+                                  int64_t text_len, int64_t B, int64_t H, int64_t S, int64_t head_dim, float eps, float q_out_scale,
+                                  int32_t rope_mode, void* kmax2, hipStream_t stream) {
+    return qknorm_rope_fwd_impl(q_in, k_in, q_out, k_out, qin_strides, kin_strides, qout_strides, kout_strides, wq, bq, wk, bk, rope_cos, rope_sin, text_len,
+                                B, H, S, head_dim, eps, q_out_scale, rope_mode, (unsigned*)kmax2, stream);
 }
 
 int32_t vgpa_qknorm_rope_bwd(const void* dq_out, const void* dk_out, const void* q_in, const void* k_in, void* dq_in, void* dk_in,
diff --git a/videogpa_amd/ops.py b/videogpa_amd/ops.py
--- a/videogpa_amd/ops.py
+++ b/videogpa_amd/ops.py
@@ -939,7 +939,15 @@
     return float((_strip_flags(ws, B * H, B, H, S) != 0).float().mean())
 
 
-def attention_fwd_raw(q, k, v, scale=None, q_prescaled=False, split_mode=None, o_pad=0, o_res=None, policy=None):
+ATTN_FUSED_PRODUCERS = True
+
+
+def attention_fwd_workspace(B, H, S, device):
+    ws_bytes = _lib.query("vgpa_attn_fwd_w1_workspace_bytes", B, H, S)
+    return torch.empty(ws_bytes, dtype=torch.uint8, device=device), ws_bytes
+
+
+def attention_fwd_raw(q, k, v, scale=None, q_prescaled=False, split_mode=None, o_pad=0, o_res=None, policy=None, kmax_ws=None):
     B, H, S, Dh = q.shape
     scale = Dh ** -0.5 if scale is None else scale
     if not q_prescaled:
@@ -948,10 +956,12 @@
     lse = torch.empty(B, H, S, dtype=torch.float32, device=q.device)
     ov = o.unflatten(-1, (H, Dh)).permute(0, 2, 1, 3)
     split_mode = ATTN_SPLIT_MODE if split_mode is None else split_mode
-    ws_bytes = _lib.query("vgpa_attn_fwd_w1_workspace_bytes", B, H, S)
-    ws = torch.empty(ws_bytes, dtype=torch.uint8, device=q.device)
+    ws, ws_bytes = attention_fwd_workspace(B, H, S, q.device) if kmax_ws is None else kmax_ws
     rv = None if o_res is None else o_res.unflatten(-1, (H, Dh)).permute(0, 2, 1, 3)
-    entry = "vgpa_attn_fwd_online_res" if (policy is not None and policy.mode == "online") else "vgpa_attn_fwd_w1_res"
+    online = policy is not None and policy.mode == "online"
+    if online and kmax_ws is not None:
+        raise ValueError("attention_fwd_raw: kmax_ws goes with the w1 forward, not with the online policy")
+    entry = "vgpa_attn_fwd_online_res" if online else ("vgpa_attn_fwd_w1_res" if kmax_ws is None else "vgpa_attn_fwd_w1_kmax")
     _timed("attn_fwd_kernel", 4.0 * S * S * Dh * B * H, lambda: _lib.call(
         entry, q, k, v, o, o_res, _res_kind(o_res), lse, _bhs_strides(q), _bhs_strides(k), _bhs_strides(v), _bhs_strides(ov), None if rv is None else _bhs_strides(rv),
         B, H, S, Dh, float(scale), int(split_mode), ws, ws_bytes, _stream()))
@@ -967,19 +977,27 @@
     scale = Dh ** -0.5 if scale is None else scale
     if not q_prescaled:
         q = prescale_q(q, scale)
-    delta = torch.empty(B, H, S, dtype=torch.float32, device=q.device)
     st = _stream()
     stats = torch.empty(B, H, 2, S, dtype=torch.float32, device=q.device)
-    _timed("attn_delta_kernel", (4.0 + (0 if o_res is None else o_res.element_size())) * B * H * S * Dh, lambda: _lib.call(
-        "vgpa_attn_bwd_prep_w1_res", o, o_res, _res_kind(o_res), do, lse, _bhs_strides(o), None if o_res is None else _bhs_strides(o_res), _bhs_strides(do),
-        delta, stats, B, H, S, Dh, st), "byte")
     split_mode = ATTN_SPLIT_MODE if split_mode is None else split_mode
     ws_bytes = _lib.query("vgpa_attn_bwd_split_workspace_bytes", B, H, S) if split_mode != 0 else 0
     ws = torch.empty(max(ws_bytes, 16), dtype=torch.uint8, device=q.device)
     wsp = ws if ws_bytes else None
-    _timed("attn_bwd_dkv_kernel", 6.0 * S * S * Dh * B * H, lambda: _lib.call(
+    dkv = lambda: _timed("attn_bwd_dkv_kernel", 6.0 * S * S * Dh * B * H, lambda: _lib.call(
         "vgpa_attn_bwd_dkv_w1", q, k, v, do, stats, dk, dv, _bhs_strides(q), _bhs_strides(k), _bhs_strides(v), _bhs_strides(do),
         _bhs_strides(dk), _bhs_strides(dv), B, H, S, Dh, float(scale), int(split_mode), wsp, ws_bytes, st))
+    if ATTN_FUSED_PRODUCERS:
+        _timed("attn_bwd_dq_kernel", 2.0 * S * S * Dh * B * H, lambda: _lib.call(
+            "vgpa_attn_bwd_dq_stats_w1", q, k, v, do, o, o_res, _res_kind(o_res), lse, None, stats, dq, _bhs_strides(q), _bhs_strides(k), _bhs_strides(v),
+            _bhs_strides(do), _bhs_strides(o), None if o_res is None else _bhs_strides(o_res), _bhs_strides(dq), B, H, S, Dh, float(scale), int(split_mode),
+            wsp, ws_bytes, st))
+        dkv()
+        return
+    delta = torch.empty(B, H, S, dtype=torch.float32, device=q.device)
+    _timed("attn_delta_kernel", (4.0 + (0 if o_res is None else o_res.element_size())) * B * H * S * Dh, lambda: _lib.call(
+        "vgpa_attn_bwd_prep_w1_res", o, o_res, _res_kind(o_res), do, lse, _bhs_strides(o), None if o_res is None else _bhs_strides(o_res), _bhs_strides(do),
+        delta, stats, B, H, S, Dh, st), "byte")
+    dkv()
     _timed("attn_bwd_dq_kernel", 2.0 * S * S * Dh * B * H, lambda: _lib.call(
         "vgpa_attn_bwd_dq_w1", q, k, v, do, lse, delta, dq, _bhs_strides(q), _bhs_strides(k), _bhs_strides(v), _bhs_strides(do),
         _bhs_strides(dq), B, H, S, Dh, float(scale), int(split_mode), wsp, ws_bytes, st))
@@ -1122,13 +1140,17 @@
         q_in, k_in, v = (qkv5[:, :, i].permute(0, 2, 1, 3) for i in range(3))
         qn = torch.empty(B, H, S, Dh, dtype=torch.bfloat16, device=qkv.device)
         kn = torch.empty_like(qn)
+        kmax_ws = None
+        if ATTN_FUSED_PRODUCERS and Dh == 64 and not (fwd_policy is not None and fwd_policy.mode == "online"):
+            kmax_ws = attention_fwd_workspace(B, H, S, qkv.device)
         _timed("qknorm_rope_fwd", 8.0 * B * H * S * Dh, lambda: _lib.call(
-            "vgpa_qknorm_rope_fwd", q_in, k_in, qn, kn, _bhs_strides(q_in), _bhs_strides(k_in), _bhs_strides(qn), _bhs_strides(kn),
-            wq, bq, wk, bk, rope_cos, rope_sin, text_len, B, H, S, Dh, float(eps), float(Dh ** -0.5 * LOG2E), int(rope_mode), _stream()), "byte")
+            "vgpa_qknorm_rope_fwd_kmax", q_in, k_in, qn, kn, _bhs_strides(q_in), _bhs_strides(k_in), _bhs_strides(qn), _bhs_strides(kn),
+            wq, bq, wk, bk, rope_cos, rope_sin, text_len, B, H, S, Dh, float(eps), float(Dh ** -0.5 * LOG2E), int(rope_mode),
+            None if kmax_ws is None else kmax_ws[0], _stream()), "byte")
         o_res = None
         if precise_delta and ctx.needs_input_grad[0]:
             o_res = torch.empty(B, S, H * Dh, dtype=torch.uint8 if precise_delta == "int8" else torch.bfloat16, device=qkv.device)
-        o, lse = attention_fwd_raw(qn, kn, v, q_prescaled=True, o_pad=o_pad, o_res=o_res, policy=fwd_policy)
+        o, lse = attention_fwd_raw(qn, kn, v, q_prescaled=True, o_pad=o_pad, o_res=o_res, policy=fwd_policy, kmax_ws=kmax_ws)
         if recompute_qk:
             ctx.save_for_backward(qkv, o, lse, wq, wk, rope_cos, rope_sin, bq, bk, o_res)
         else:
```

New measurement: 0.4470 pair-steps/s, median of 6. No clear change (+0.4%).
